# InternetMaximalism/plonky2_bn254

Hardware: AMD Instinct MI355X
Metric: G1 scalar-mul STARK proofs/sec (256-bit scalars) (higher is better)
Workload: dtype u64 (Goldilocks p = 2^64-2^32+1; BN254 Fq as 10x26-bit Montgomery limbs); 1 GPU; configs[1]: batch of 1024 G1 scalar-muls on 1 GPU per step = 8 proofs x 128 instances, 2^16 rows, W=781, standard_fast_config; instances_per_proof=128, steps_in_flight=4, parallelism=1 GPU, no collective

## Files before the change

include/bn254_stark.h:

```cpp
#ifndef BN254_STARK_H
#define BN254_STARK_H

#include <stddef.h>
#include <stdint.h>

#ifdef __cplusplus
extern "C" {
#endif

#define BN254S_ABI_VERSION 1

enum {
  BN254S_OK = 0,
  BN254S_E_INVALID_ARG = -1,
  BN254S_E_HIP = -2,
  BN254S_E_OOM = -3,
  BN254S_E_INVALID_POINT = -4,
  BN254S_E_UNSUPPORTED = -5,
  BN254S_E_TRANSCRIPT = -6,
  BN254S_E_INTERNAL = -7,
  BN254S_E_VERIFY = -8
};

typedef struct bn254s_ctx bn254s_ctx;
// ... 30 lines not shown
                       const uint64_t* offset, size_t n_total, size_t per_proof, bn254s_proof** proofs_out);

typedef struct bn254s_batch bn254s_batch;
int bn254s_prove_batch_begin(bn254s_ctx* ctx, int kind, const bn254s_params* params, const uint64_t* scalars, const uint64_t* x,
                             const uint64_t* offset, size_t n_total, size_t per_proof, bn254s_proof** proofs_out,
                             bn254s_batch** handle);
int bn254s_prove_batch_end(bn254s_batch* handle);

int bn254s_prove_batch_multi(bn254s_ctx** ctxs, size_t n_ctx, int kind, const bn254s_params* params, const uint64_t* scalars,
                             const uint64_t* x, const uint64_t* offset, size_t n_total, size_t per_proof, bn254s_proof** proofs);

int bn254s_prove_g2(bn254s_ctx* ctx, const bn254s_params* params, const uint64_t* scalars, const uint64_t* x,
                    const uint64_t* offset, size_t n, bn254s_proof** out);
int bn254s_prove_fq_exp(bn254s_ctx* ctx, const bn254s_params* params, const uint64_t* scalars ,
                        const uint64_t* x , size_t n, bn254s_proof** out);

int bn254s_proof_words(const bn254s_proof* p, const uint64_t** data, size_t* len);
enum {
  BN254S_SEC_TRACE_CAP = 0,
  BN254S_SEC_AUX_CAP = 1,
  BN254S_SEC_QUOTIENT_CAP = 2,
  BN254S_SEC_LOCAL_VALUES = 3,
  BN254S_SEC_NEXT_VALUES = 4,
  BN254S_SEC_AUX_POLYS = 5,
  BN254S_SEC_AUX_POLYS_NEXT = 6,
  BN254S_SEC_CTL_ZS_FIRST = 7,
  BN254S_SEC_QUOTIENT_POLYS = 8,
  BN254S_SEC_FRI_CAPS = 9,
  BN254S_SEC_QUERY_ROUNDS = 10,
  BN254S_SEC_FINAL_POLY = 11,
  BN254S_SEC_POW_WITNESS = 12,
  BN254S_SEC_INIT_CHALLENGER_STATE = 13,
  BN254S_SEC_COUNT = 14
};
int bn254s_proof_section(const bn254s_proof* p, int id, const uint64_t** data, size_t* len);
int bn254s_proof_degree_bits(const bn254s_proof* p);
int bn254s_proof_outputs(const bn254s_proof* p, const uint64_t** data, size_t* len);
int bn254s_proof_stage_ms(const bn254s_proof* p, const float** ms, size_t* n_stages);
const char* bn254s_stage_name(size_t stage);
size_t bn254s_proof_serialize(const bn254s_proof* p, uint8_t* buf, size_t cap);
void bn254s_proof_free(bn254s_proof* p);

int bn254s_verify(bn254s_ctx* ctx, int kind, const bn254s_params* params, uint32_t degree_bits, const uint64_t* words,
                  size_t n_words, const uint64_t* scalars, const uint64_t* x, const uint64_t* offset, const uint64_t* outputs,
                  size_t n);
int bn254s_verify_host(int kind, const bn254s_params* params, uint32_t degree_bits, const uint64_t* words, size_t n_words,
                       const uint64_t* scalars, const uint64_t* x, const uint64_t* offset, const uint64_t* outputs, size_t n,
                       char* err_buf, size_t err_cap);

int bn254s_verify_batch(bn254s_ctx* ctx, int kind, const bn254s_params* params, uint32_t degree_bits, const uint64_t* const* words,
                        size_t n_words, const uint64_t* scalars, const uint64_t* x, const uint64_t* offset, const uint64_t* outputs,
                        const size_t* n_jobs, size_t n_proofs, int32_t* status, char* err, size_t err_stride);

int bn254s_ctl_values(int kind, const uint64_t* scalars, const uint64_t* x, const uint64_t* offset, const uint64_t* outputs,
                      size_t n, uint64_t* in_rows, uint64_t* out_rows);

int bn254s_map_to_g2(bn254s_ctx* ctx, const bn254s_params* params, const uint64_t* u, const uint64_t* offsets, size_t n,
                     uint64_t* out_points, uint64_t* fq_jobs, uint64_t* g2_jobs, bn254s_proof** fq_proofs,
                     bn254s_proof** g2_proofs);

int bn254s_hash_to_fq2(const uint64_t* input, size_t len, uint64_t* out );
int bn254s_hash_to_fq2_batch(bn254s_ctx* ctx, const uint64_t* inputs, size_t n, size_t len, uint64_t* out);

int bn254s_g1_msm_chain(bn254s_ctx* ctx, const uint64_t* scalars , const uint64_t* x ,
                        const uint64_t* offset , size_t n, uint64_t* offsets_out, uint64_t* result );
int bn254s_g1_msm(bn254s_ctx* ctx, const bn254s_params* params, const uint64_t* scalars, const uint64_t* x,
                  const uint64_t* offset, size_t n, size_t per_proof, uint64_t* result, uint64_t* offsets_out,
                  bn254s_proof** proofs);
int bn254s_g2_msm_chain(bn254s_ctx* ctx, const uint64_t* scalars , const uint64_t* x ,
                        const uint64_t* offset , size_t n, uint64_t* offsets_out ,
                        uint64_t* result );
int bn254s_g2_msm(bn254s_ctx* ctx, const bn254s_params* params, const uint64_t* scalars, const uint64_t* x,
                  const uint64_t* offset, size_t n, size_t per_proof, uint64_t* result, uint64_t* offsets_out,
                  bn254s_proof** proofs);

int bn254s_g1_recover_from_x_batch(bn254s_ctx* ctx, const uint64_t* xs , size_t n,
                                   uint64_t* points_out , uint8_t* flags_out ,
                                   uint64_t* fq_jobs );
int bn254s_g1_recover_from_x(bn254s_ctx* ctx, const bn254s_params* params, const uint64_t* xs, size_t n, size_t per_proof,
                             uint64_t* points_out, uint8_t* flags_out, uint64_t* fq_jobs ,
                             bn254s_proof** fq_proofs);
int bn254s_g2_recover_from_x_batch(bn254s_ctx* ctx, const uint64_t* xs ,
                                   const uint8_t* sgns , size_t n,
                                   uint64_t* points_out , uint8_t* flags_out ,
                                   uint64_t* fq_jobs );
int bn254s_g2_recover_from_x(bn254s_ctx* ctx, const bn254s_params* params, const uint64_t* xs, const uint8_t* sgns, size_t n,
                             size_t per_proof, uint64_t* points_out, uint8_t* flags_out, uint64_t* fq_jobs ,
                             bn254s_proof** fq_proofs);
int bn254s_g2_subgroup_check_batch(bn254s_ctx* ctx, const uint64_t* points , size_t n,
                                   uint8_t* flags_out );
int bn254s_g2_subgroup_check(bn254s_ctx* ctx, const bn254s_params* params, const uint64_t* points ,
                             const uint64_t* offsets , size_t n, size_t per_proof, uint8_t* flags_out ,
                             uint64_t* g2_jobs , bn254s_proof** g2_proofs);
int bn254s_g2_clear_cofactor_batch(bn254s_ctx* ctx, const uint64_t* points , size_t n,
                                   uint64_t* images_out , uint8_t* finite_out );
int bn254s_g2_clear_cofactor(bn254s_ctx* ctx, const bn254s_params* params, const uint64_t* points ,
                             const uint64_t* offsets , size_t n, size_t per_proof, uint64_t* images_out ,
                             uint8_t* finite_out , uint64_t* g2_jobs ,
                             bn254s_proof** g2_proofs);
int bn254s_map_to_g2_batch(bn254s_ctx* ctx, const uint64_t* u , size_t n,
                           uint64_t* out_points );
int bn254s_hash_to_g2_batch(bn254s_ctx* ctx, const uint64_t* inputs , size_t n, size_t len,
                            uint64_t* out_points );
int bn254s_hash_to_fq(const uint64_t* input, size_t len, uint64_t* out );
int bn254s_hash_to_fq_batch(bn254s_ctx* ctx, const uint64_t* inputs, size_t n, size_t len, uint64_t* out );
int bn254s_map_to_g1_batch(bn254s_ctx* ctx, const uint64_t* u , size_t n,
                           uint64_t* out_points , uint8_t* sq_flags ,
                           uint64_t* fq_jobs );
int bn254s_hash_to_g1_batch(bn254s_ctx* ctx, const uint64_t* inputs , size_t n, size_t len,
                            uint64_t* out_points );
int bn254s_map_to_g1(bn254s_ctx* ctx, const bn254s_params* params, const uint64_t* u , size_t n, size_t per_proof,
                     uint64_t* out_points , uint8_t* sq_flags ,
                     uint64_t* fq_jobs , bn254s_proof** fq_proofs );
int bn254s_job_outputs_batch(bn254s_ctx* ctx, int kind, const uint64_t* scalars , const uint64_t* x,
                             const uint64_t* offset, size_t n, uint64_t* outputs_out ,
                             uint8_t* finite_out );
int bn254s_job_outputs(bn254s_ctx* ctx, int kind, const bn254s_params* params, const uint64_t* scalars, const uint64_t* x,
                       const uint64_t* offset, size_t n, size_t per_proof, uint64_t* outputs_out, bn254s_proof** proofs_out);
int bn254s_commit_values(bn254s_ctx* ctx, const uint64_t* values, size_t ncols, uint64_t* coeffs, uint64_t* lde,
                         uint64_t* cap);
int bn254s_bench_ntt(bn254s_ctx* ctx, size_t ncols, int iters, float* ms);
int bn254s_bench_ntt_clock(bn254s_ctx* ctx, size_t ncols, int iters, float* ms, float* mhz, float* mhz_min);
int bn254s_bench_issue(bn254s_ctx* ctx, float* ns_per_issue, float* mhz);
int bn254s_bench_copy(bn254s_ctx* ctx, size_t words, int iters);
int bn254s_bench_leafhash(bn254s_ctx* ctx, size_t ncols, int log_leaves, int iters, float* ms);
int bn254s_poseidon_permute(bn254s_ctx* ctx, uint64_t* states, size_t n);
int bn254s_selftest_field(bn254s_ctx* ctx, const uint64_t* a, const uint64_t* b, size_t n, uint64_t* out);
int bn254s_selftest_poseidon(bn254s_ctx* ctx, int variant, uint64_t* states, size_t n);
int bn254s_selftest_leaf_hash(bn254s_ctx* ctx, const uint64_t* data, size_t ncols, int log_leaves, int kernel, int chunk_cols,
                              uint64_t* digests);
int bn254s_selftest_fq_inv(bn254s_ctx* ctx, const uint64_t* x, size_t n, uint64_t* out);
int bn254s_selftest_fq(bn254s_ctx* ctx, int group, const uint64_t* in, size_t n, uint64_t* out);
int bn254s_selftest_logup(bn254s_ctx* ctx, const uint64_t* trace, size_t rows, int ncols, int rc_begin, int n_rc, int table_col,
                          int freq_col, const uint64_t betas[2], uint64_t* out);
int bn254s_selftest_acc(bn254s_ctx* ctx, const uint64_t* values, const uint64_t* weights, size_t T, size_t rows, uint64_t* out);
int bn254s_selftest_openings(bn254s_ctx* ctx, const uint64_t* coeffs, int npolys, int log_r, const uint64_t zeta[2],
                             const uint64_t zeta_next[2], uint64_t* out);
int bn254s_selftest_fri_combine(bn254s_ctx* ctx, int mode, int W, int n_rc, int n_ctl, size_t n, const uint64_t* cols,
                                const uint64_t* aux_in, const uint64_t* points, uint64_t* out);
int bn254s_selftest_fri_fold(bn254s_ctx* ctx, const uint64_t* in, int log_m, uint64_t shift, const uint64_t beta[2], uint64_t* out);
int bn254s_selftest_fri_rows(bn254s_ctx* ctx, const uint64_t* lde, int ncols, int log_n, int h, size_t k0, size_t rows,
                             const uint32_t* indices, int nq, uint64_t* window, uint64_t* gathered);
#define BN254S_VERIFY_RECORD_HEAD 34
int bn254s_selftest_verify_front(int kind, const bn254s_params* params, uint32_t degree_bits, const uint64_t* words, size_t n_words,
                                 uint64_t* record_out, size_t record_cap);
int bn254s_selftest_query_round(bn254s_ctx* ctx, int kind, const bn254s_params* params, uint32_t degree_bits,
                                const uint64_t* const* words, size_t n_words, const uint64_t* records, size_t n_proofs,
                                size_t chunk_proofs, int32_t* codes_out);
const char* bn254s_selftest_query_text(int n_layers, int code);
int bn254s_selftest_verify_batch_ms(bn254s_ctx* ctx, float ms_out[5]);
#define BN254S_PLAN_WORDS 54
int bn254s_selftest_proof_plan(int kind, size_t n, const bn254s_params* params, uint64_t dev_total_bytes, int force_split,
                               int force_lowmem, int force_stream, int stream_win_log, uint64_t* out, char* err, size_t err_len);
int bn254s_generate_trace(bn254s_ctx* ctx, int kind, const uint64_t* scalars, const uint64_t* x, const uint64_t* offset,
                          size_t n, uint32_t min_rows_log2, uint64_t* trace_out, uint64_t* outputs);
int bn254s_g1_generate_trace(bn254s_ctx* ctx, const uint64_t* scalars, const uint64_t* x, const uint64_t* offset,
                             size_t n, uint32_t min_rows_log2, uint64_t* trace_out, uint64_t* outputs);

#ifdef __cplusplus
}
#endif
#endif
```

plonky2_bn254_amd/__init__.py:

```python
import os as _os

_os.environ.setdefault("GPU_MAX_HW_QUEUES", "16")

from .lib import Context, Proof, load_library, LibraryMissing, VerifyError, default_params, proof_plan, proof_words, prove_batch_multi, query_round, query_text, verify_g1_msm, verify_g1_recover, verify_g2_clear_cofactor, verify_g2_msm, verify_g2_recover, verify_batch_host, verify_front, verify_g2_subgroup, verify_host, verify_job_outputs, verify_map_to_g1
```

plonky2_bn254_amd/csrc/capi.hip:

```cpp
#include <algorithm>
#include <cstring>
#include "proven_jobs.h"
#include "merkle.h"
#include "trace_g1.h"
#include "fq_selftest.h"
#include "aux.h"
#include "poseidon_dev.h"

void ntt_module_warm();
void merkle_module_warm();
void aux_module_warm();
void fri_module_warm();
void quotient_g1_module_warm();
void quotient_g2fq_module_warm();
void trace_g1_module_warm();
void trace_g2fq_module_warm();
void prover_module_warm();

extern "C" {

int bn254s_abi_version(void) { return BN254S_ABI_VERSION; }

void bn254s_params_default(bn254s_params* p) {
  p->struct_size = sizeof(bn254s_params);
  p->security_bits = 100;
  p->num_challenges = 2;
  p->rate_bits = 1;
  p->cap_height = 4;
  p->pow_bits = 16;
  p->arity_bits = 4;
  p->final_poly_bits = 5;
  p->num_queries = 84;
  p->min_rows_log2 = 16;
}

__attribute__((constructor)) static void bn254s_runtime_defaults() { setenv("GPU_MAX_HW_QUEUES", "16", 0); }


int bn254s_ctx_create(int device_id, bn254s_ctx** out) {
  if (!out) return BN254S_E_INVALID_ARG;
  *out = nullptr;
  int ndev = 0;
  if (hipGetDeviceCount(&ndev) != hipSuccess || device_id < 0 || device_id >= ndev) return BN254S_E_HIP;
  if (const char* e = getenv("BN254S_SYNC"))
    if (!strcmp(e, "blocking")) (void)hipSetDeviceFlags(hipDeviceScheduleBlockingSync);
  (void)hipGetLastError();
  if (hipSetDevice(device_id) != hipSuccess) return BN254S_E_HIP;
  bn254s_ctx* c = new bn254s_ctx();
  c->device = device_id;
  merkle_set_throughput_mode(getenv("BN254S_COOP_MAX_NODES") ? atol(getenv("BN254S_COOP_MAX_NODES")) : -1,
                             getenv("BN254S_MERKLE_LEVEL_ASM") ? atoi(getenv("BN254S_MERKLE_LEVEL_ASM")) : -1);
  if (const char* e = getenv("BN254S_BIG_CAP")) c->big_cap = std::max(1, atoi(e));
  if (const char* e = getenv("BN254S_SCHED_FIFO")) c->big_fifo = atoi(e) != 0;
  if (const char* e = getenv("BN254S_NTT_CONVOY")) c->big_convoy = std::max(0, atoi(e));
  if (const char* e = getenv("BN254S_HASH_SPLIT")) c->hash_split = std::min(8, std::max(1, atoi(e)));
  c->big_cost[BIG_NTT] = c->big_cap;
  const char* cost_env[3] = {"BN254S_BIG_COST_NTT", "BN254S_BIG_COST_EXCL", "BN254S_BIG_COST_HASH"};
  for (int k = 0; k < 3; k++) {
    if (const char* e = getenv(cost_env[k])) c->big_cost[k] = atoi(e);
    c->big_cost[k] = std::min(c->big_cap, std::max(0, c->big_cost[k]));
  }
  c->big_cost[BIG_HASH_PART] = std::max(1, c->big_cost[BIG_HASH] / c->hash_split);
  if (hipStreamCreateWithFlags(&c->stream, hipStreamNonBlocking) != hipSuccess) {
    delete c;
    return BN254S_E_HIP;
  }
  if (ntt_tables_init(&c->ntt) != 0) {
    delete c;
    return BN254S_E_OOM;
  }
  {
    void* h = nullptr;
    if (hipHostMalloc(&h, 256 << 10) == hipSuccess) {
      (void)hipMemcpyAsync(h, c->ntt.twmat_fwd, 256 << 10, hipMemcpyDeviceToHost, c->stream);
      (void)hipStreamSynchronize(c->stream);
      hipHostFree(h);
    }
  }
  ntt_module_warm();
  merkle_module_warm();
  aux_module_warm();
  fri_module_warm();
  quotient_g1_module_warm();
  quotient_g2fq_module_warm();
  trace_g1_module_warm();
  trace_g2fq_module_warm();
  prover_module_warm();
  *out = c;
  return BN254S_OK;
}

void bn254s_ctx_destroy(bn254s_ctx* c) {
  if (!c) return;
  hipSetDevice(c->device);
  c->workers.shutdown();
  hipStreamSynchronize(c->stream);
  for (Slot* s : c->slots) {
    hipStreamSynchronize(s->st);
    s->mem.release();
    if (s->pinned) hipHostFree(s->pinned);
    for (auto& e : s->events) hipEventDestroy(e);
    hipStreamDestroy(s->st);
    delete s;
  }
  for (auto& kv : c->tall) {
    ntt_tall_tables_free(kv.second);
    delete kv.second;
  }
  for (auto& kv : c->split) {
    ntt_split_tables_free(kv.second);
    delete kv.second;
  }
  c->release();
  ntt_tables_free(&c->ntt);
  hipStreamDestroy(c->stream);
  delete c;
}

int bn254s_ctx_trim(bn254s_ctx* c) {
  if (!c) return BN254S_E_INVALID_ARG;
  HIP_TRY(c, hipSetDevice(c->device));
  auto give_back = [&](size_t i) {
    if (i < c->n_slots_now()) c->slot(i)->mem.release();
  };
  if (c->workers.busy.empty()) {
    for (size_t i = 0; i < c->n_slots_now(); i++) give_back(i);
  } else {
    c->workers.for_idle_slots(give_back);
  }
  bool idle;
  {
    std::lock_guard<std::mutex> lk(c->workers.mu);
    idle = c->workers.n_busy == 0 && c->workers.q.empty();
  }
  if (idle) {
    HIP_TRY(c, hipStreamSynchronize(c->stream));
    c->release();
  }
  return BN254S_OK;
}

const char* bn254s_last_error(const bn254s_ctx* c) { return c ? c->err.c_str() : "null context"; }

int bn254s_commit_values(bn254s_ctx* c, const uint64_t* values, size_t ncols, uint64_t* coeffs, uint64_t* lde,
                         uint64_t* cap) {
  if (!c || !values || ncols == 0) return BN254S_E_INVALID_ARG;
  HIP_TRY(c, hipSetDevice(c->device));
  const size_t N = NTT_N;
  u64* d_vals = c->words("cv.vals", ncols * N);
  u64* d_tmp = c->words("cv.tmp", 3 * ncols * N);
  u64* d_lde = c->words("cv.lde", ncols * 2 * N);
  u64* d_tree = c->words("cv.tree", merkle_tree_digests(17, 4) * 4);
  if (!d_vals || !d_tmp || !d_lde || !d_tree) return BN254S_E_OOM;
  HIP_TRY(c, hipMemcpyAsync(d_vals, values, ncols * N * 8, hipMemcpyHostToDevice, c->stream));
  ntt_inverse_lde(&c->ntt, d_vals, d_vals, d_lde, d_tmp, d_tmp + ncols * N, (int)ncols, c->stream);
  merkle_build(d_lde, 1, 2 * N, (int)ncols, 17, 4, d_tree, c->stream);
  HIP_TRY(c, hipGetLastError());
  if (coeffs) HIP_TRY(c, hipMemcpyAsync(coeffs, d_vals, ncols * N * 8, hipMemcpyDeviceToHost, c->stream));
  if (lde) HIP_TRY(c, hipMemcpyAsync(lde, d_lde, ncols * 2 * N * 8, hipMemcpyDeviceToHost, c->stream));
  if (cap)
    HIP_TRY(c, hipMemcpyAsync(cap, d_tree + 4 * merkle_level_offset(17, 13), 16 * 32, hipMemcpyDeviceToHost, c->stream));
  HIP_TRY(c, hipStreamSynchronize(c->stream));
  return BN254S_OK;
}

__global__ void k_fill_pseudo(u64* p, size_t n, u64 seed) {
  size_t i = (size_t)blockIdx.x * blockDim.x + threadIdx.x;
  if (i >= n) return;
  u64 z = seed + i * 0x9E3779B97F4A7C15ULL;
  z = (z ^ (z >> 30)) * 0xBF58476D1CE4E5B9ULL;
  z = (z ^ (z >> 27)) * 0x94D049BB133111EBULL;
  z ^= z >> 31;
  p[i] = z >= GL_P ? z - GL_P : z;
}

int bn254s_bench_ntt(bn254s_ctx* c, size_t ncols, int iters, float* ms) {
  if (!c || !ms || ncols == 0 || iters <= 0) return BN254S_E_INVALID_ARG;
  HIP_TRY(c, hipSetDevice(c->device));
  const size_t N = NTT_N;
  u64* d_vals = c->words("cv.vals", ncols * N);
  u64* d_tmp = c->words("cv.tmp", 3 * ncols * N);
  u64* d_lde = c->words("cv.lde", ncols * 2 * N);
  if (!d_vals || !d_tmp || !d_lde) return BN254S_E_OOM;
  size_t n = ncols * N;
  k_fill_pseudo<<<(unsigned)((n + 255) / 256), 256, 0, c->stream>>>(d_vals, n, 0x1234);
  hipEvent_t e0, e1;
  HIP_TRY(c, hipEventCreate(&e0));
  HIP_TRY(c, hipEventCreate(&e1));
  ntt_inverse_lde(&c->ntt, d_vals, d_vals, d_lde, d_tmp, d_tmp + n, (int)ncols, c->stream);
  HIP_TRY(c, hipEventRecord(e0, c->stream));
  for (int it = 0; it < iters; it++) ntt_inverse_lde(&c->ntt, d_vals, d_vals, d_lde, d_tmp, d_tmp + n, (int)ncols, c->stream);
  HIP_TRY(c, hipEventRecord(e1, c->stream));
  HIP_TRY(c, hipEventSynchronize(e1));
  float t = 0;
  HIP_TRY(c, hipEventElapsedTime(&t, e0, e1));
  *ms = t / iters;
  hipEventDestroy(e0);
  hipEventDestroy(e1);
  HIP_TRY(c, hipGetLastError());
  return BN254S_OK;
}

__global__ __launch_bounds__(64) void k_clock_probe(unsigned long long* __restrict__ samples, const int* __restrict__ stop, int max_samples,
                                                    int* __restrict__ n_taken) {
  if (threadIdx.x != 0) return;
  int i = 0;
  for (; i < max_samples; i++) {
    samples[2 * i] = __builtin_readcyclecounter();
    samples[2 * i + 1] = __builtin_amdgcn_s_memrealtime();
    if (__hip_atomic_load(stop, __ATOMIC_RELAXED, __HIP_MEMORY_SCOPE_AGENT)) {
      i++;
      break;
    }
    __builtin_amdgcn_s_sleep(127);
    __builtin_amdgcn_s_sleep(127);
    __builtin_amdgcn_s_sleep(127);
  }
  *n_taken = i;
}
__global__ __launch_bounds__(256) void k_issue_probe(u64* out) {
  for (int i = 0; i < 2048; i++) {
    asm volatile(
        "v_lshl_add_u64 v[40:41], v[40:41], 0, v[48:49]\n v_lshl_add_u64 v[42:43], v[42:43], 0, v[48:49]\n"
        "v_lshl_add_u64 v[44:45], v[44:45], 0, v[48:49]\n v_lshl_add_u64 v[46:47], v[46:47], 0, v[48:49]\n"
        "v_lshl_add_u64 v[40:41], v[40:41], 0, v[48:49]\n v_lshl_add_u64 v[42:43], v[42:43], 0, v[48:49]\n"
        "v_lshl_add_u64 v[44:45], v[44:45], 0, v[48:49]\n v_lshl_add_u64 v[46:47], v[46:47], 0, v[48:49]\n"
        "v_lshl_add_u64 v[40:41], v[40:41], 0, v[48:49]\n v_lshl_add_u64 v[42:43], v[42:43], 0, v[48:49]\n"
        "v_lshl_add_u64 v[44:45], v[44:45], 0, v[48:49]\n v_lshl_add_u64 v[46:47], v[46:47], 0, v[48:49]\n"
        "v_lshl_add_u64 v[40:41], v[40:41], 0, v[48:49]\n v_lshl_add_u64 v[42:43], v[42:43], 0, v[48:49]\n"
        "v_lshl_add_u64 v[44:45], v[44:45], 0, v[48:49]\n v_lshl_add_u64 v[46:47], v[46:47], 0, v[48:49]\n"
        "v_lshl_add_u64 v[40:41], v[40:41], 0, v[48:49]\n v_lshl_add_u64 v[42:43], v[42:43], 0, v[48:49]\n"
        "v_lshl_add_u64 v[44:45], v[44:45], 0, v[48:49]\n v_lshl_add_u64 v[46:47], v[46:47], 0, v[48:49]\n"
        "v_lshl_add_u64 v[40:41], v[40:41], 0, v[48:49]\n v_lshl_add_u64 v[42:43], v[42:43], 0, v[48:49]\n"
        "v_lshl_add_u64 v[44:45], v[44:45], 0, v[48:49]\n v_lshl_add_u64 v[46:47], v[46:47], 0, v[48:49]\n"
        "v_lshl_add_u64 v[40:41], v[40:41], 0, v[48:49]\n v_lshl_add_u64 v[42:43], v[42:43], 0, v[48:49]\n"
        "v_lshl_add_u64 v[44:45], v[44:45], 0, v[48:49]\n v_lshl_add_u64 v[46:47], v[46:47], 0, v[48:49]\n"
        "v_lshl_add_u64 v[40:41], v[40:41], 0, v[48:49]\n v_lshl_add_u64 v[42:43], v[42:43], 0, v[48:49]\n"
        "v_lshl_add_u64 v[44:45], v[44:45], 0, v[48:49]\n v_lshl_add_u64 v[46:47], v[46:47], 0, v[48:49]\n" ::
            : "v40", "v41", "v42", "v43", "v44", "v45", "v46", "v47");
  }
  u32 a;
  asm volatile("v_mov_b32 %0, v40" : "=v"(a));
  out[(size_t)blockIdx.x * blockDim.x + threadIdx.x] = a;
}
int bn254s_bench_issue(bn254s_ctx* c, float* ns_per_issue, float* mhz) {
  if (!c || !ns_per_issue || !mhz) return BN254S_E_INVALID_ARG;
  HIP_TRY(c, hipSetDevice(c->device));
  hipDeviceProp_t prop;
  HIP_TRY(c, hipGetDeviceProperties(&prop, c->device));
  const int simds = prop.multiProcessorCount * 4, blocks = simds * 8 / 4;
  const int MAXS = 20000;
  u64* d_out = c->words("iss.out", (size_t)blocks * 256);
  unsigned long long* d_s = (unsigned long long*)c->words("clk.samples", 2 * (size_t)MAXS + 2);
  if (!d_out || !d_s) return BN254S_E_OOM;
  int* d_flags = (int*)(d_s + 2 * (size_t)MAXS);
  hipStream_t ps = nullptr;
  HIP_TRY(c, hipStreamCreateWithFlags(&ps, hipStreamNonBlocking));
  HIP_TRY(c, hipMemsetAsync(d_flags, 0, 8, c->stream));
  HIP_TRY(c, hipStreamSynchronize(c->stream));
  hipEvent_t e0, e1;
  HIP_TRY(c, hipEventCreate(&e0));
  HIP_TRY(c, hipEventCreate(&e1));
  k_clock_probe<<<1, 64, 0, ps>>>(d_s, d_flags, MAXS, d_flags + 1);
  const int reps = 12;
  for (int i = 0; i < 4; i++) k_issue_probe<<<blocks, 256, 0, c->stream>>>(d_out);
  HIP_TRY(c, hipEventRecord(e0, c->stream));
  for (int i = 0; i < reps; i++) k_issue_probe<<<blocks, 256, 0, c->stream>>>(d_out);
  HIP_TRY(c, hipEventRecord(e1, c->stream));
  (void)hipMemsetAsync(d_flags, 1, 1, c->stream);
  HIP_TRY(c, hipStreamSynchronize(c->stream));
  (void)hipStreamSynchronize(ps);
  hipStreamDestroy(ps);
  float t = 0;
  HIP_TRY(c, hipEventElapsedTime(&t, e0, e1));
  hipEventDestroy(e0);
  hipEventDestroy(e1);
  *ns_per_issue = (float)((double)t * 1e6 / reps / (2048.0 * 32 * 8));
  std::vector<unsigned long long> h(2 * (size_t)MAXS + 2);
  HIP_TRY(c, hipMemcpy(h.data(), d_s, h.size() * 8, hipMemcpyDeviceToHost));
  const int n = ((const int*)&h[2 * (size_t)MAXS])[1];
  *mhz = 0;
  if (n >= 8) {
    const int lo = n / 4;
    const double dt = (double)(h[2 * (size_t)(n - 1) + 1] - h[2 * (size_t)lo + 1]), dc = (double)(h[2 * (size_t)(n - 1)] - h[2 * (size_t)lo]);
    if (dt > 0) *mhz = (float)(dc / dt * 100.0);
  }
  return BN254S_OK;
}

int bn254s_bench_ntt_clock(bn254s_ctx* c, size_t ncols, int iters, float* ms, float* mhz, float* mhz_min) {
  if (!c || !ms || !mhz || ncols == 0 || iters <= 0) return BN254S_E_INVALID_ARG;
  HIP_TRY(c, hipSetDevice(c->device));
  const int MAXS = 20000;
  unsigned long long* d_s = (unsigned long long*)c->words("clk.samples", 2 * (size_t)MAXS + 2);
  if (!d_s) return BN254S_E_OOM;
// ... 263 lines not shown
```

plonky2_bn254_amd/csrc/ctx.h:

```cpp
#pragma once
#include <string>
#include <vector>
#include <map>
#include <cstdio>
#include <mutex>
#include <condition_variable>
#include <chrono>
#include <deque>
#include <functional>
#include <thread>
#include <atomic>
#include <hip/hip_runtime.h>
#include "../../include/bn254_stark.h"
#include "gl_dev.h"
#include "ntt.h"

struct BufPool {
  std::map<std::string, std::pair<void*, size_t>> pool;
  std::string err;
  void* buf(const std::string& name, size_t bytes) {
    auto it = pool.find(name);
    if (it != pool.end() && it->second.second >= bytes) return it->second.first;
    if (it != pool.end()) {
      hipFree(it->second.first);
      pool.erase(it);
    }
    void* p = nullptr;
    if (hipMalloc(&p, bytes) != hipSuccess) {
      (void)hipGetLastError();
      err = "hipMalloc failed for " + name + " (" + std::to_string(bytes) + " bytes)";
      return nullptr;
    }
    pool[name] = {p, bytes};
    return p;
  }
  u64* words(const std::string& name, size_t n) { return (u64*)buf(name, n * 8); }
  bool has(const std::string& name) const { return pool.find(name) != pool.end(); }
  void drop(const std::string& name) {
    auto it = pool.find(name);
    if (it == pool.end()) return;
    hipFree(it->second.first);
    pool.erase(it);
  }
  void release() {
    for (auto& kv : pool) hipFree(kv.second.first);
    pool.clear();
  }
};

struct Slot {
  hipStream_t st = nullptr;
  BufPool mem;
  void* pinned = nullptr;
  size_t pinned_bytes = 0;
  std::vector<hipEvent_t> events;
};

enum { BIG_NTT = 0, BIG_EXCL = 1, BIG_HASH = 2, BIG_HASH_PART = 3 };

struct WorkPool {
  std::mutex mu;
  std::condition_variable cv, done_cv;
  std::deque<std::function<void(size_t)>> q;
  std::vector<std::thread> th;
  std::vector<char> busy;
  bool stop = false;
  size_t limit = 0, n_busy = 0;
  size_t n_waiting = 0, completions = 0;
  std::mutex retry_mu;
  std::atomic<int> in_flight{0};
  void start(size_t n, int device) {
    std::lock_guard<std::mutex> lk(mu);
    limit = n;
    if (busy.size() < n) busy.resize(n, 0);
    while (th.size() < n) {
      th.emplace_back([this, device]() {
        (void)hipSetDevice(device);
        for (;;) {
          std::function<void(size_t)> f;
          size_t s = 0;
          {
            std::unique_lock<std::mutex> lk2(mu);
            auto free_slot = [&]() -> size_t {
              for (size_t i = 0; i < limit && i < busy.size(); i++)
                if (!busy[i]) return i;
              return (size_t)-1;
            };
            cv.wait(lk2, [&] { return (stop && q.empty()) || (!q.empty() && n_busy < limit && free_slot() != (size_t)-1); });
            if (q.empty()) return;
            f = std::move(q.front());
            q.pop_front();
            s = free_slot();
            busy[s] = 1;
            n_busy++;
            in_flight.store((int)n_busy, std::memory_order_relaxed);
          }
          f(s);
          {
            std::lock_guard<std::mutex> lk3(mu);
            busy[s] = 0;
            n_busy--;
            in_flight.store((int)n_busy, std::memory_order_relaxed);
            completions++;
          }
          cv.notify_one();
          done_cv.notify_all();
        }
      });
    }
  }
  void push(std::function<void(size_t)> f) {
    {
      std::lock_guard<std::mutex> lk(mu);
      q.push_back(std::move(f));
    }
    cv.notify_one();
  }
  template <class G>
  void for_idle_slots(G g) {
    std::vector<size_t> idle;
    {
      std::lock_guard<std::mutex> lk(mu);
      for (size_t i = 0; i < busy.size(); i++)
        if (!busy[i]) {
          busy[i] = 2;
          idle.push_back(i);
        }
    }
    for (size_t i : idle) g(i);
    {
      std::lock_guard<std::mutex> lk(mu);
      for (size_t i : idle) busy[i] = 0;
    }
    cv.notify_all();
  }
  size_t active() {
    std::lock_guard<std::mutex> lk(mu);
    return n_busy - n_waiting;
  }
  size_t completions_now() {
    std::lock_guard<std::mutex> lk(mu);
    return completions;
  }
  void wait_for_a_completion(size_t c0) {
    std::unique_lock<std::mutex> lk(mu);
    n_waiting++;
    done_cv.wait_for(lk, std::chrono::seconds(60), [&] { return completions != c0; });
    n_waiting--;
  }
  void shutdown() {
    {
      std::lock_guard<std::mutex> lk(mu);
      stop = true;
    }
    cv.notify_all();
    for (auto& t : th) t.join();
    th.clear();
  }
};

struct bn254s_ctx : BufPool {
  int device = 0;
  hipStream_t stream = nullptr;
  NttTables ntt;
  std::vector<Slot*> slots;
  WorkPool workers;
  std::map<unsigned, NttTallTables*> tall;
  std::map<unsigned, NttSplitTables*> split;
  std::mutex big_mu;
  std::condition_variable big_cv;
  int big_cap = 12, big_cost[4] = {12, 2, 4, 2}, big_used = 0;
  int hash_split = 1;
  bool big_fifo = true;
  struct BigWaiter {
    unsigned long id;
    int cls;
  };
  std::deque<BigWaiter> big_q;
  unsigned long big_next_id = 0;
  int big_convoy = 4, big_convoy_run = 0;
  bool big_last_was_ntt = false;
  void big_lock(int cls) {
    std::unique_lock<std::mutex> lk(big_mu);
    if (big_fifo) {
      const unsigned long my = big_next_id++;
      big_q.push_back({my, cls});
      big_cv.wait(lk, [&] {
        if (big_q.front().id == my) {
          if (big_used + big_cost[cls] > big_cap) return false;
          if (big_last_was_ntt && cls != BIG_NTT && big_convoy_run < big_convoy)
            for (const BigWaiter& w : big_q)
              if (w.cls == BIG_NTT) return false;
          return true;
        }
        if (cls != BIG_NTT || !big_last_was_ntt || big_used != 0 || big_convoy_run >= big_convoy) return false;
        if (big_q.front().cls == BIG_NTT) return false;
        for (const BigWaiter& w : big_q) {
          if (w.cls == BIG_NTT) return w.id == my;
        }
        return false;
      });
      const bool in_order = big_q.front().id == my;
      for (auto it = big_q.begin(); it != big_q.end(); ++it)
        if (it->id == my) {
          big_q.erase(it);
          break;
        }
      if (in_order) big_convoy_run = 0;
      else big_convoy_run++;
      big_last_was_ntt = false;
      big_used += big_cost[cls];
      lk.unlock();
      big_cv.notify_all();
      return;
    }
    big_cv.wait(lk, [&] { return big_used + big_cost[cls] <= big_cap; });
    big_used += big_cost[cls];
  }
  void big_unlock(int cls) {
    {
      std::lock_guard<std::mutex> lk(big_mu);
      big_used -= big_cost[cls];
      big_last_was_ntt = cls == BIG_NTT && big_used == 0;
    }
    big_cv.notify_all();
  }
  static constexpr size_t MAX_SLOTS = 64;
  std::mutex slots_mu, err_mu;
  float vb_ms[5] = {0, 0, 0, 0, 0};
  bn254s_ctx() { slots.reserve(MAX_SLOTS); }
  void set_err(const std::string& e) {
    std::lock_guard<std::mutex> lk(err_mu);
    err = e;
  }
  size_t n_slots_now() {
    std::lock_guard<std::mutex> lk(slots_mu);
    return slots.size();
  }
  Slot* slot(size_t i) {
    if (i >= MAX_SLOTS) return nullptr;
    std::lock_guard<std::mutex> lk(slots_mu);
    while (slots.size() <= i) {
      Slot* s = new Slot();
      if (hipStreamCreateWithFlags(&s->st, hipStreamNonBlocking) != hipSuccess) {
        delete s;
        return nullptr;
      }
      slots.push_back(s);
    }
    return slots[i];
  }
};

#define HIP_TRY(ctx, call)                                                                  \
  do {                                                                                      \
    hipError_t e_ = (call);                                                                 \
    if (e_ != hipSuccess) {                                                                 \
      (ctx)->set_err(std::string(#call) + ": " + hipGetErrorString(e_));                    \
      return BN254S_E_HIP;                                                                  \
    }                                                                                       \
  } while (0)
```

plonky2_bn254_amd/csrc/ntt.h:

```cpp
#pragma once
#include <vector>
#include "gl_dev.h"

static constexpr size_t NTT_N = 65536;

struct NttTables {
  u64 *tw256_fwd = nullptr, *tw256_inv = nullptr;
  u64 *twmat_fwd = nullptr, *twmat_inv = nullptr;
  u64* twmat_inv_ninv = nullptr;
  u64* coset_pow[2] = {nullptr, nullptr};
  u64* coset_inv_pow[2] = {nullptr, nullptr};
  u64 n_inv = 0;
};

int ntt_tables_init(NttTables* T);
void ntt_tables_free(NttTables* T);
void ntt_inverse(const NttTables* T, const u64* values, u64* coeffs, u64* tmp, int ncols, hipStream_t s);
void ntt_coset_inverse(const NttTables* T, int h, const u64* values, u64* coeffs, u64* tmp, int ncols, hipStream_t s);
void ntt_lde(const NttTables* T, const u64* coeffs, u64* lde, u64* tmp, int ncols, hipStream_t s);
void ntt_inverse_lde(const NttTables* T, const u64* values, u64* coeffs, u64* lde, u64* tmp, u64* tmp2, int ncols, hipStream_t s);
void ntt_coset_forward_natural(const NttTables* T, int h, const u64* coeffs, u64* values, u64* tmp, int ncols, hipStream_t s);

struct NttTallTables {
  unsigned log_n = 0;
  u64* wn_inv_pow = nullptr;
  u64* wn_pow_br = nullptr;
  u64* block_coset_pow[2] = {nullptr, nullptr};
  u64 shift[2] = {0, 0};
  u64 r_inv = 0;
};
int ntt_tall_tables_init(NttTallTables* T, unsigned log_n, u64 base_shift = GL_GEN);
void ntt_tall_tables_free(NttTallTables* T);
void ntt_inverse_tall(const NttTables* T, const NttTallTables* TT, const u64* values, u64* coeffs, u64* tmp, int ncols,
                      hipStream_t s);
void ntt_coset_inverse_tall(const NttTables* T, const NttTallTables* TT, int h, const u64* values, u64* coeffs, u64* tmp, int ncols,
                            hipStream_t s);
void ntt_inverse_lde_tall(const NttTables* T, const NttTallTables* TT, const u64* values, u64* coeffs, u64* lde, u64* tmp, int ncols,
                          hipStream_t s);
void ntt_lde_tall(const NttTables* T, const NttTallTables* TT, const u64* coeffs, u64* lde, u64* tmp, int ncols, hipStream_t s,
                  int coset_mask = 3);

struct NttSplitTables {
  unsigned log_n = 0;
  u64 *fwd_lo = nullptr, *fwd_hi = nullptr, *inv_lo = nullptr, *inv_hi = nullptr;
  u64 shift[2] = {0, 0};
  u64 half = 0;
};
int ntt_split_tables_init(NttSplitTables* S, unsigned log_n);
void ntt_split_tables_free(NttSplitTables* S);
void ntt_split_inverse(const NttSplitTables* S, const u64* values, u64* halves, int ncols, hipStream_t s);
void ntt_split_forward(const NttSplitTables* S, const u64* eo, u64* lde, size_t lde_stride, int ncols, hipStream_t s, int coset_mask = 3);
void ntt_coset_inverse_split(const NttTables* T, const NttTallTables* TT, const NttSplitTables* S, int h, const u64* values, u64* coeffs,
                             u64* tmp, int ncols, hipStream_t s);

static constexpr int FIELD_SELFTEST_OUTS = 17;
void field_selftest(const u64* a, const u64* b, u64* out, size_t n, hipStream_t s);
```

plonky2_bn254_amd/csrc/ntt.hip:

```cpp
#include "gl_dev.h"
#include "gl_asm.h"
#include "ntt.h"

#if defined(__HIP_DEVICE_COMPILE__) && defined(BN254S_NTT_PRIO) && BN254S_NTT_PRIO > 0
#define NTT_KERNEL_PRIO() __builtin_amdgcn_s_setprio(BN254S_NTT_PRIO)
#else
#define NTT_KERNEL_PRIO() ((void)0)
#endif

template <bool INV, int SPAN, int G, int J>
__device__ __forceinline__ void bfly16(u64* x) {
  constexpr int E = J * (8 / SPAN);
  constexpr int S0 = E == 0 ? 0 : (!INV ? 12 * E : 192 - 12 * E);
  constexpr bool NEG0 = S0 >= 96;
  constexpr int S1 = NEG0 ? S0 - 96 : S0;
  constexpr bool RIGHT = S1 > 64;
  constexpr bool NEG = NEG0 != RIGHT;
  u64 s, d;
  gl_bfly_asm<NEG>(x[G + J], x[G + J + SPAN], s, d);
  x[G + J] = s;
  if constexpr (S1 == 0) x[G + J + SPAN] = d;
  else if constexpr (RIGHT) x[G + J + SPAN] = gl_shr_small_asm<96 - S1>(d);
  else x[G + J + SPAN] = gl_shl_asm<S1>(d);
}
// ... 122 lines not shown
    __syncthreads();
    ulonglong2* o16 = reinterpret_cast<ulonglong2*>(ocol + (size_t)br4(blockIdx.x) * 16 * 256);
#pragma unroll
    for (int i = 0; i < 8; i++) {
      const int piece = i * 256 + t;
      o16[piece] = stage[(piece >> 7) * STAGE_ROW + ((piece >> 3) & 15) * 9 + (piece & 7)];
    }
  } else {
#pragma unroll
    for (int kb = 0; kb < 16; kb++) {
      int k = k1 + 256 * (ka + 16 * kb);
      u64 v = x[br4(kb)];
      if (post) v = gl_mul_asm(v, post[k]);
      else if (post_scalar != 1) v = gl_mul_asm(v, post_scalar);
      ocol[k] = v;
    }
  }
}

template <int NPARK>
__global__ __launch_bounds__(256, NPARK ? 4 : 3) void k_ntt_intt2_lde1(const u64* __restrict__ in, size_t in_stride, u64* __restrict__ coef,
                                                        size_t coef_stride, u64* __restrict__ y0, u64* __restrict__ y1,
                                                        size_t y_stride, const u64* __restrict__ tw256_inv,
                                                        const u64* __restrict__ pre0, const u64* __restrict__ pre1,
                                                        const u64* __restrict__ twmat, const u64* __restrict__ tw256_fwd,
                                                        unsigned log_r) {
  NTT_KERNEL_PRIO();
  __shared__ u32 lds[LDS_TILE_WORDS];
  __shared__ u64 park[NPARK ? NPARK * 256 : 1];
  u64 c[16];
  const int t = threadIdx.x;
  int g = t & 15, d = t >> 4;
  const u64* col = in + col_offset(blockIdx.y, log_r, in_stride);
  u64 x[16];
  {
    const int k1_load = blockIdx.x * 16 + d;
#pragma unroll
    for (int m = 0; m < 16; m++) x[m] = col[k1_load * 256 + g + 16 * m];
  }
  dft256_tile<true, 2>(x, lds, tw256_inv, d, g);
  const int i2 = blockIdx.x * 16 + d;
  u64* ocol = coef + col_offset(blockIdx.y, log_r, coef_stride);
#pragma unroll
  for (int kb = 0; kb < 16; kb++) {
    c[kb] = x[br4(kb)];
    ocol[i2 + 256 * (g + 16 * kb)] = c[kb];
    if (kb >= 16 - NPARK) park[(kb - (16 - NPARK)) * 256 + t] = c[kb];
  }
#pragma unroll 1
  for (int h = 0; h < 2; h++) {
    const u64* __restrict__ pre = h ? pre1 : pre0;
    u64* ycol = (h ? y1 : y0) + col_offset(blockIdx.y, log_r, y_stride);
    asm volatile("" : "+v"(g), "+v"(d));
#pragma unroll
    for (int m = 0; m < 16; m++) {
      x[m] = gl_mul_asm(m >= 16 - NPARK ? park[(m - (16 - NPARK)) * 256 + t] : c[m], pre[(g + 16 * m) * 256 + i2]);
      if ((m & 3) == 3) __builtin_amdgcn_sched_barrier(0);
    }
    __syncthreads();
    dft256_tile<false, 0>(x, lds, tw256_fwd, d, g);
#pragma unroll
    for (int kb = 0; kb < 16; kb++) {
      int k1 = g + 16 * kb;
      ycol[k1 * 256 + i2] = gl_mul_asm(x[br4(kb)], twmat[k1 * 256 + i2]);
      if ((kb & 3) == 3) __builtin_amdgcn_sched_barrier(0);
    }
  }
}

static void fill_pow_table(std::vector<u64>& t, u64 base, size_t n, u64 first = 1) {
  t.resize(n);
  u64 v = first;
  for (size_t i = 0; i < n; i++) {
    t[i] = v;
    v = gl_mul(v, base);
  }
}

int ntt_tables_init(NttTables* T) {
  const size_t N = NTT_N;
  std::vector<u64> h;
  auto upload = [&](u64** dst, const std::vector<u64>& src) -> int {
    if (hipMalloc((void**)dst, src.size() * 8) != hipSuccess) return -1;
    if (hipMemcpy(*dst, src.data(), src.size() * 8, hipMemcpyHostToDevice) != hipSuccess) return -1;
    return 0;
  };
  u64 wN = gl_root_of_unity(16), wNi = gl_inv(wN);
  u64 w256 = gl_root_of_unity(8), w256i = gl_inv(w256);
  fill_pow_table(h, w256, 256);
  if (upload(&T->tw256_fwd, h)) return -1;
  fill_pow_table(h, w256i, 256);
  if (upload(&T->tw256_inv, h)) return -1;
  for (int inv = 0; inv < 2; inv++) {
    u64 w = inv ? wNi : wN;
    h.resize(N);
    u64 wk = 1;
    for (int k1 = 0; k1 < 256; k1++) {
      u64 v = 1;
      for (int i2 = 0; i2 < 256; i2++) {
        h[k1 * 256 + i2] = v;
        v = gl_mul(v, wk);
      }
      wk = gl_mul(wk, w);
    }
    if (upload(inv ? &T->twmat_inv : &T->twmat_fwd, h)) return -1;
    if (inv) {
      const u64 ninv0 = gl_inv((u64)N);
      for (auto& v : h) v = gl_mul(v, ninv0);
      if (upload(&T->twmat_inv_ninv, h)) return -1;
    }
  }
  u64 w2N = gl_root_of_unity(17);
  u64 shifts[2] = {GL_GEN, gl_mul(GL_GEN, w2N)};
  u64 ninv = gl_inv((u64)N);
  for (int hh = 0; hh < 2; hh++) {
    fill_pow_table(h, shifts[hh], N);
    if (upload(&T->coset_pow[hh], h)) return -1;
    fill_pow_table(h, gl_inv(shifts[hh]), N, ninv);
    if (upload(&T->coset_inv_pow[hh], h)) return -1;
  }
  T->n_inv = ninv;
  return 0;
}

void ntt_tables_free(NttTables* T) {
  hipFree(T->tw256_fwd);
  hipFree(T->tw256_inv);
  hipFree(T->twmat_fwd);
  hipFree(T->twmat_inv);
  hipFree(T->twmat_inv_ninv);
  for (int h = 0; h < 2; h++) {
    hipFree(T->coset_pow[h]);
    hipFree(T->coset_inv_pow[h]);
  }
}

void ntt_inverse(const NttTables* T, const u64* values, u64* coeffs, u64* tmp, int ncols, hipStream_t s) {
  dim3 grid(16, ncols), block(256);
  k_ntt_pass1<true><<<grid, block, 0, s>>>(values, NTT_N, tmp, NTT_N, nullptr, T->twmat_inv, T->tw256_inv, 0);
  k_ntt_pass2<true, false><<<grid, block, 0, s>>>(tmp, NTT_N, coeffs, NTT_N, nullptr, T->n_inv, T->tw256_inv, 0);
}
void ntt_coset_inverse(const NttTables* T, int h, const u64* values, u64* coeffs, u64* tmp, int ncols, hipStream_t s) {
  dim3 grid(16, ncols), block(256);
  k_ntt_pass1<true><<<grid, block, 0, s>>>(values, NTT_N, tmp, NTT_N, nullptr, T->twmat_inv, T->tw256_inv, 0);
  k_ntt_pass2<true, false><<<grid, block, 0, s>>>(tmp, NTT_N, coeffs, NTT_N, T->coset_inv_pow[h], 1, T->tw256_inv, 0);
}
void ntt_lde(const NttTables* T, const u64* coeffs, u64* lde, u64* tmp, int ncols, hipStream_t s) {
  dim3 grid(16, ncols), block(256);
  for (int h = 0; h < 2; h++) {
    k_ntt_pass1<false><<<grid, block, 0, s>>>(coeffs, NTT_N, tmp, NTT_N, T->coset_pow[h], T->twmat_fwd, T->tw256_fwd, 0);
    k_ntt_pass2<false, true><<<grid, block, 0, s>>>(tmp, NTT_N, lde + (size_t)h * NTT_N, 2 * NTT_N, nullptr, 1, T->tw256_fwd, 0);
  }
}
void ntt_inverse_lde(const NttTables* T, const u64* values, u64* coeffs, u64* lde, u64* tmp, u64* tmp2, int ncols, hipStream_t s) {
  dim3 grid(16, ncols), block(256);
  u64* y0 = tmp2;
  u64* y1 = tmp2 + (size_t)ncols * NTT_N;
  k_ntt_pass1<true><<<grid, block, 0, s>>>(values, NTT_N, tmp, NTT_N, nullptr, T->twmat_inv_ninv, T->tw256_inv, 0);
  k_ntt_intt2_lde1<8><<<grid, block, 0, s>>>(tmp, NTT_N, coeffs, NTT_N, y0, y1, NTT_N, T->tw256_inv, T->coset_pow[0],
                                          T->coset_pow[1], T->twmat_fwd, T->tw256_fwd, 0);
  k_ntt_pass2<false, true><<<grid, block, 0, s>>>(y0, NTT_N, lde, 2 * NTT_N, nullptr, 1, T->tw256_fwd, 0);
  k_ntt_pass2<false, true><<<grid, block, 0, s>>>(y1, NTT_N, lde + NTT_N, 2 * NTT_N, nullptr, 1, T->tw256_fwd, 0);
}
void ntt_coset_forward_natural(const NttTables* T, int h, const u64* coeffs, u64* values, u64* tmp, int ncols, hipStream_t s) {
  dim3 grid(16, ncols), block(256);
  k_ntt_pass1<false><<<grid, block, 0, s>>>(coeffs, NTT_N, tmp, NTT_N, T->coset_pow[h], T->twmat_fwd, T->tw256_fwd, 0);
  k_ntt_pass2<false, false><<<grid, block, 0, s>>>(tmp, NTT_N, values, NTT_N, nullptr, 1, T->tw256_fwd, 0);
}


__device__ __forceinline__ u64 mul_2exp3(u64 x, int e) {
  switch (e) {
    case 0: return x;
    case 1: return gl_mul_2exp<3>(x);
    case 2: return gl_mul_2exp<6>(x);
    case 3: return gl_mul_2exp<9>(x);
    case 4: return gl_mul_2exp<12>(x);
    case 5: return gl_mul_2exp<15>(x);
    case 6: return gl_mul_2exp<18>(x);
    case 7: return gl_mul_2exp<21>(x);
    case 8: return gl_mul_2exp<24>(x);
    case 9: return gl_mul_2exp<27>(x);
    case 10: return gl_mul_2exp<30>(x);
    case 11: return gl_mul_2exp<33>(x);
    case 12: return gl_mul_2exp<36>(x);
    case 13: return gl_mul_2exp<39>(x);
    case 14: return gl_mul_2exp<42>(x);
    case 15: return gl_mul_2exp<45>(x);
    case 16: return gl_mul_2exp<48>(x);
    case 17: return gl_mul_2exp<51>(x);
    case 18: return gl_mul_2exp<54>(x);
    case 19: return gl_mul_2exp<57>(x);
    case 20: return gl_mul_2exp<60>(x);
    case 21: return gl_mul_2exp<63>(x);
    case 22: return gl_mul_2exp<66>(x);
    case 23: return gl_mul_2exp<69>(x);
    case 24: return gl_mul_2exp<72>(x);
    case 25: return gl_mul_2exp<75>(x);
    case 26: return gl_mul_2exp<78>(x);
    case 27: return gl_mul_2exp<81>(x);
    case 28: return gl_mul_2exp<84>(x);
    case 29: return gl_mul_2exp<87>(x);
    case 30: return gl_mul_2exp<90>(x);
    case 31: return gl_mul_2exp<93>(x);
    case 32: return gl_mul_2exp<96>(x);
    case 33: return gl_mul_2exp<99>(x);
    case 34: return gl_mul_2exp<102>(x);
    case 35: return gl_mul_2exp<105>(x);
    case 36: return gl_mul_2exp<108>(x);
    case 37: return gl_mul_2exp<111>(x);
    case 38: return gl_mul_2exp<114>(x);
    case 39: return gl_mul_2exp<117>(x);
    case 40: return gl_mul_2exp<120>(x);
    case 41: return gl_mul_2exp<123>(x);
    case 42: return gl_mul_2exp<126>(x);
    case 43: return gl_mul_2exp<129>(x);
    case 44: return gl_mul_2exp<132>(x);
    case 45: return gl_mul_2exp<135>(x);
    case 46: return gl_mul_2exp<138>(x);
    case 47: return gl_mul_2exp<141>(x);
    case 48: return gl_mul_2exp<144>(x);
    case 49: return gl_mul_2exp<147>(x);
    case 50: return gl_mul_2exp<150>(x);
    case 51: return gl_mul_2exp<153>(x);
    case 52: return gl_mul_2exp<156>(x);
    case 53: return gl_mul_2exp<159>(x);
    case 54: return gl_mul_2exp<162>(x);
    case 55: return gl_mul_2exp<165>(x);
    case 56: return gl_mul_2exp<168>(x);
    case 57: return gl_mul_2exp<171>(x);
    case 58: return gl_mul_2exp<174>(x);
    case 59: return gl_mul_2exp<177>(x);
    case 60: return gl_mul_2exp<180>(x);
    case 61: return gl_mul_2exp<183>(x);
    case 62: return gl_mul_2exp<186>(x);
    default: return gl_mul_2exp<189>(x);
  }
}
template <int LOGR, bool INV>
__device__ __forceinline__ void dft_small(u64* x) {
  constexpr int R = 1 << LOGR;
#pragma unroll
  for (int s = 0; s < LOGR; s++) {
    const int span = R >> (s + 1);
#pragma unroll
    for (int g0 = 0; g0 < R; g0 += 2 * span) {
#pragma unroll
      for (int jj = 0; jj < span; jj++) {
        u64 a = x[g0 + jj], b = x[g0 + jj + span];
        x[g0 + jj] = gl_add(a, b);
        int e = (jj << s) * (64 >> LOGR);
        if (INV) e = (64 - e) & 63;
        x[g0 + jj + span] = mul_2exp3(gl_sub(a, b), e);
      }
    }
  }
}
__device__ __forceinline__ constexpr int brn(int v, int bits) {
  int r = 0;
  for (int i = 0; i < bits; i++) r |= ((v >> i) & 1) << (bits - 1 - i);
  return r;
}

template <int LOGR>
__global__ __launch_bounds__(256) void k_ntt_outer_inv(const u64* __restrict__ in, u64* __restrict__ out, size_t N,
                                                       const u64* __restrict__ wn_inv_pow , u64 r_inv) {
  constexpr int R = 1 << LOGR;
  const size_t i2 = (size_t)blockIdx.x * blockDim.x + threadIdx.x;
  const u64* c = in + (size_t)blockIdx.y * N;
  u64* o = out + (size_t)blockIdx.y * N;
  u64 x[R];
#pragma unroll
  for (int i1 = 0; i1 < R; i1++) x[i1] = c[(size_t)i1 * NTT_N + i2];
  dft_small<LOGR, true>(x);
  const u64 w = wn_inv_pow[i2];
  u64 f = r_inv;
#pragma unroll
  for (int k1 = 0; k1 < R; k1++) {
    o[(size_t)k1 * NTT_N + i2] = gl_mul(x[brn(k1, LOGR)], f);
    f = gl_mul(f, w);
  }
}

template <int LOGR>
__global__ __launch_bounds__(256) void k_ntt_outer_fwd(const u64* __restrict__ z, size_t N, u64* __restrict__ out,
                                                       size_t out_stride, const u64* __restrict__ wn_pow_br ,
                                                       u64 shift) {
  constexpr int R = 1 << LOGR;
  const size_t p = (size_t)blockIdx.x * blockDim.x + threadIdx.x;
  const u64* c = z + (size_t)blockIdx.y * N;
  u64 x[R];
  const u64 b = gl_mul(shift, wn_pow_br[p]);
  u64 f = 1;
#pragma unroll
  for (int i1 = 0; i1 < R; i1++) {
    u64 v = c[(size_t)i1 * NTT_N + p];
    x[i1] = i1 ? gl_mul(v, f) : v;
    f = gl_mul(f, b);
  }
  dft_small<LOGR, false>(x);
  constexpr int CH = R < 16 ? R : 16;
  constexpr int U = CH / 2;
  constexpr int PITCH = U + 1;
  __shared__ ulonglong2 stage[256 * PITCH];
  const int t = threadIdx.x;
  ulonglong2* o16 = reinterpret_cast<ulonglong2*>(out + (size_t)blockIdx.y * out_stride + (size_t)blockIdx.x * 256 * R);
#pragma unroll
  for (int c0 = 0; c0 < R; c0 += CH) {
    if (c0) __syncthreads();
#pragma unroll
    for (int u = 0; u < U; u++) {
      ulonglong2 w2;
      w2.x = x[c0 + 2 * u];
      w2.y = x[c0 + 2 * u + 1];
// ... 264 lines not shown
```

plonky2_bn254_amd/csrc/prover.hip:

```cpp
#include <algorithm>
#include <atomic>
#include <cstring>
#include <thread>
#include "ctx.h"
#include "trace_g1.h"
#include "trace_g2fq.h"
#include "aux.h"
#include "merkle.h"
#include "quotient.h"
#include "fri.h"
#include "transcript.h"
#include "prover.h"
#include "proof_plan.h"

template <class L>
static StarkShape make_shape(bool input_has_a, int n_constraints) {
  StarkShape s;
  s.W = L::W;
  s.rc_begin = L::RC_BEGIN;
  s.rc_end = L::RC_END;
  s.table_col = L::RANGE;
  s.freq_col = L::FREQ;
  s.n_ctl = 2;
  s.n_constraints = n_constraints;
  memset(&s.ctl, 0, sizeof(s.ctl));
  int m = 0;
  for (int i = 0; i < L::PL; i++, m++) { s.ctl.col_start[0][m] = L::B + i; s.ctl.col_bits[0][m] = 1; }
  if (input_has_a)
    for (int i = 0; i < L::PL; i++, m++) { s.ctl.col_start[0][m] = L::A + i; s.ctl.col_bits[0][m] = 1; }
  for (int k = 0; k < 16; k++, m++) { s.ctl.col_start[0][m] = L::BITS + 16 * k; s.ctl.col_bits[0][m] = 16; }
  s.ctl.col_start[0][m] = L::TIMESTAMP; s.ctl.col_bits[0][m] = 1; m++;
  s.ctl.ncols[0] = m;
  s.ctl.filter_col[0] = L::FLAGS + 0;
  m = 0;
  for (int i = 0; i < L::PL; i++, m++) { s.ctl.col_start[1][m] = L::SUM + i; s.ctl.col_bits[1][m] = 1; }
  s.ctl.col_start[1][m] = L::TIMESTAMP; s.ctl.col_bits[1][m] = 1; m++;
  s.ctl.ncols[1] = m;
  s.ctl.filter_col[1] = L::FLAGS + 1;
  return s;
}
static int fq_generate_trace_no_offset(const u64* d_scalars, const u64* d_x, const u64*, size_t n, u64* d_trace, size_t N,
                                       u64* d_scratch, u64* d_outputs, int* d_err, hipStream_t st, bool with_range) {
  return fq_generate_trace_device(d_scalars, d_x, n, d_trace, N, d_scratch, d_outputs, d_err, st, with_range);
}
const StarkKind& stark_kind(int kind) {
  static const StarkKind kinds[3] = {
      {make_shape<G1L>(true, 1111), 8, true, g1_trace_scratch_words, g1_generate_trace_device, g1_quotient_mz_blocks, g1_quotient_launch},
      {make_shape<G2L>(true, 1693), 16, true, g2_trace_scratch_words, g2_generate_trace_device, g2_quotient_mz_blocks, g2_quotient_launch},
      {make_shape<FQL>(false, 770), 4, false, fq_trace_scratch_words, fq_generate_trace_no_offset, fq_quotient_mz_blocks, fq_quotient_launch}};
  return kinds[kind];
}

enum { ST_TRACE = 0, ST_TRACE_NTT, ST_TRACE_MERKLE, ST_AUX, ST_AUX_NTT, ST_AUX_MERKLE, ST_QUOTIENT, ST_QUOTIENT_COMMIT,
       ST_OPENINGS, ST_FRI, ST_TOTAL, ST_COUNT };
static const char* STAGE_NAMES[ST_COUNT] = {"trace_gen", "trace_ntt", "trace_merkle", "aux_columns", "aux_ntt", "aux_merkle",
                                            "quotient", "quotient_commit", "openings", "fri", "total"};

struct bn254s_proof {
  std::vector<u64> words, outputs;
  size_t sec_off[BN254S_SEC_COUNT + 1] = {0};
  int degree_bits = 0;
  float stage_ms[ST_COUNT] = {0};
};

std::vector<int> fri_arities(const bn254s_params& P, int degree_bits) {
  std::vector<int> a;
  int d = degree_bits;
  while (d > (int)P.final_poly_bits && d + (int)P.rate_bits - (int)P.arity_bits >= (int)P.cap_height) {
    a.push_back(P.arity_bits);
    d -= P.arity_bits;
  }
  return a;
}

__global__ __launch_bounds__(256) void k_quotient_chunks(const u64* __restrict__ ab, u64* __restrict__ out, size_t N, u64 inv2,
                                                         u64 inv2c) {
  size_t i = (size_t)blockIdx.x * blockDim.x + threadIdx.x;
  if (i >= N) return;
  int a = blockIdx.y;
  u64 A = ab[(size_t)(a * 2 + 0) * N + i], B = ab[(size_t)(a * 2 + 1) * N + i];
  out[(size_t)(a * 2 + 0) * N + i] = gl_mul(gl_add(A, B), inv2);
  out[(size_t)(a * 2 + 1) * N + i] = gl_mul(gl_sub(A, B), inv2c);
}

#define CHK(call)                                              \
  do {                                                         \
    hipError_t e_ = (call);                                    \
    if (e_ != hipSuccess) {                                    \
      err = std::string(#call) + ": " + hipGetErrorString(e_); \
      return BN254S_E_HIP;                                     \
    }                                                          \
  } while (0)

static const NttTallTables* get_tall_tables(bn254s_ctx* c, unsigned log_n, bool half_of_split = false) {
  static std::mutex mu;
  std::lock_guard<std::mutex> lk(mu);
  const unsigned key = log_n + (half_of_split ? 100 : 0);
  auto it = c->tall.find(key);
  if (it != c->tall.end()) return it->second;
  NttTallTables* t = new NttTallTables();
  if (ntt_tall_tables_init(t, log_n, half_of_split ? gl_mul(GL_GEN, GL_GEN) : GL_GEN) != 0) {
    delete t;
    return nullptr;
  }
  c->tall[key] = t;
  return t;
}
static const NttSplitTables* get_split_tables(bn254s_ctx* c, unsigned log_n) {
  static std::mutex mu;
  std::lock_guard<std::mutex> lk(mu);
  auto it = c->split.find(log_n);
  if (it != c->split.end()) return it->second;
  NttSplitTables* t = new NttSplitTables();
  if (ntt_split_tables_init(t, log_n) != 0) {
    delete t;
    return nullptr;
  }
  c->split[log_n] = t;
  return t;
}

struct BigSection {
  bn254s_ctx* c;
  hipStream_t st;
  int cls;
  BigSection(bn254s_ctx* c_, hipStream_t st_, int cls_) : c(c_), st(st_), cls(cls_) { c->big_lock(cls); }
  ~BigSection() {
    hipStreamSynchronize(st);
    c->big_unlock(cls);
  }
};

static int get_point_tables(bn254s_ctx* c, unsigned log_n, QPointTables& pt) {
  static std::mutex mu;
  std::lock_guard<std::mutex> lk(mu);
  std::string key = "pt." + std::to_string(log_n);
  bool fresh = !c->has(key);
  size_t M2 = (size_t)2 << log_n;
  u64* p = c->words(key, 3 * M2);
  if (!p) return BN254S_E_OOM;
  if (fresh) {
    quotient_point_tables(p, p + M2, p + 2 * M2, log_n, c->stream);
    if (hipStreamSynchronize(c->stream) != hipSuccess) return BN254S_E_HIP;
  }
  pt.x = p;
  pt.lfirst = p + M2;
  pt.llast = p + 2 * M2;
  return 0;
}

struct Workspace {
  Slot* sl = nullptr;
  const ProofPlan* pl = nullptr;
  u64 *in, *tvals, *tcoef, *hist, *tmp, *ldechunk, *sponge, *comb, *tlde, *trees, *avals, *acoef, *alde, *scr, *quot, *tabs, *open,
      *fri, *fritrees, *qout;
  int* err;
  unsigned long long* pow;
  u32* qidx;
  u64 *ttree, *atree, *qtree;
  u64 *qv, *ab, *qcoef, *qlde, *qpart;
  u64 *W, *mzt, *apow;
  size_t cap_off;
  u64 *tw = nullptr, *aw = nullptr, *wpt = nullptr, *qrows = nullptr;
  int begin_windows(std::string& err);
};

static int workspace_acquire(Slot& sl, const ProofPlan& pl, Workspace& ws, std::string& err) {
  BufPool& mem = sl.mem;
  const PlanBuffers& b = pl.words;
  const bool stream = pl.stream, lowmem = pl.lowmem;
  ws.sl = &sl;
  ws.pl = &pl;
  if (lowmem) {
    mem.drop("acoef");
    mem.drop("alde");
  }
  ws.in = mem.words("in", b.in);
  ws.tvals = mem.words("tvals", b.tvals);
  ws.tcoef = mem.words("tcoef", b.tcoef);
  ws.hist = mem.words("hist", b.hist);
  ws.tmp = mem.words("tmp", b.tmp);
  mem.drop("win");
  if (stream) {
    mem.drop("tlde");
    mem.drop("alde");
    mem.drop("acoef");
  } else {
    mem.drop("ldechunk");
    mem.drop("sponge");
  }
  ws.ldechunk = stream ? mem.words("ldechunk", b.ldechunk) : nullptr;
  ws.sponge = stream ? mem.words("sponge", b.sponge) : nullptr;
  ws.comb = mem.words("comb", b.comb);
  ws.tlde = stream ? ws.ldechunk : mem.words("tlde", b.tlde);
  ws.trees = mem.words("trees", b.trees);
  ws.avals = mem.words("avals", b.avals);
  ws.acoef = lowmem ? ws.avals : mem.words("acoef", b.acoef);
  ws.alde = stream ? ws.ldechunk : lowmem ? ws.tvals : mem.words("alde", b.alde);
  ws.scr = mem.words("scratch", b.scratch);
  ws.quot = mem.words("quot", b.quot);
  ws.tabs = mem.words("tabs", b.tabs);
  ws.open = mem.words("open", b.open);
  ws.fri = mem.words("fri", b.fri);
  ws.fritrees = mem.words("fritrees", b.fritrees);
  ws.qout = mem.words("qout", b.qout);
  if (sl.pinned_bytes < pl.pinned_bytes) {
    if (sl.pinned) hipHostFree(sl.pinned);
    sl.pinned = nullptr;
    sl.pinned_bytes = 0;
    CHK(hipHostMalloc(&sl.pinned, pl.pinned_bytes));
    sl.pinned_bytes = pl.pinned_bytes;
  }
  if (!ws.hist || !ws.in || !ws.tvals || !ws.tcoef || !ws.tmp || !ws.tlde || !ws.trees || !ws.avals || !ws.acoef || !ws.alde ||
      !ws.scr || !ws.quot || !ws.tabs || !ws.open || !ws.fri || !ws.fritrees || !ws.qout || !ws.comb ||
      (stream && (!ws.ldechunk || !ws.sponge))) {
    err = mem.err;
    mem.release();
    return BN254S_E_OOM;
  }
  {
    static const size_t reserve = (size_t)(getenv("BN254S_MEM_RESERVE_MB") ? atol(getenv("BN254S_MEM_RESERVE_MB")) : 6144) << 20;
    size_t free_b = 0, total_b = 0;
    if (hipMemGetInfo(&free_b, &total_b) == hipSuccess && free_b < reserve) {
      err = "device memory: " + std::to_string(free_b >> 20) + " MB would be left free, below the reserve of " +
            std::to_string(reserve >> 20) + " MB kept for the runtime's own allocations";
      mem.release();
      return BN254S_E_OOM;
    }
  }
  const size_t N = pl.N, M2 = pl.M2;
  const int NQ = ProofPlan::NQ;
  ws.err = (int*)(ws.in + pl.in_words);
  ws.pow = (unsigned long long*)(ws.in + pl.in_words + 2);
  ws.qidx = (u32*)(ws.qout + pl.n_q());
  ws.ttree = ws.trees;
  ws.atree = ws.trees + pl.tree_words;
  ws.qtree = ws.trees + 2 * pl.tree_words;
  ws.qv = ws.quot;
  ws.ab = ws.quot + (size_t)NQ * N;
  ws.qcoef = ws.quot + (size_t)2 * NQ * N;
  ws.qlde = ws.quot + (size_t)3 * NQ * N;
  ws.qpart = ws.qlde + (size_t)NQ * M2;
  ws.W = ws.tabs;
  ws.mzt = ws.tabs + QUOTIENT_W_WORDS(pl.K);
  ws.apow = ws.mzt + QUOTIENT_MZT_WORDS;
  ws.cap_off = 4 * merkle_level_offset(pl.log_m2, pl.log_m2 - pl.P.cap_height);
  return BN254S_OK;
}

int Workspace::begin_windows(std::string& err) {
  BufPool& mem = sl->mem;
  const size_t WROWS = pl->WROWS;
  CHK(hipStreamSynchronize(sl->st));
  mem.drop("tvals");
  tvals = nullptr;
  u64* win = mem.words("win", pl->words.win);
  if (!win) {
    err = mem.err;
    mem.release();
    return BN254S_E_OOM;
  }
  tw = win;
  aw = win + (size_t)pl->W * WROWS;
  wpt = aw + (size_t)pl->A * WROWS;
  qrows = wpt + 3 * WROWS;
  return BN254S_OK;
}

struct Transforms {
  static constexpr int CH = ProofPlan::CH;
  bn254s_ctx* c;
  hipStream_t st;
  const NttTallTables* TT;
  const NttSplitTables* SP;
  const ProofPlan& pl;
  u64 *tmp, *ldechunk, *sponge;
  u64* eo() const { return tmp; }
  u64* ntmp() const { return tmp + (size_t)CH * 2 * pl.N; }

  void commit_ntt(const u64* vals, u64* coef, u64* lde, int nc) const {
    const size_t N = pl.N, M2 = pl.M2;
    if (pl.log_s) {
      for (int c0 = 0; c0 < nc; c0 += CH) {
        const int cn = std::min(CH, nc - c0);
        ntt_split_inverse(SP, vals + (size_t)c0 * N, coef + (size_t)c0 * N, cn, st);
        ntt_inverse_lde_tall(&c->ntt, TT, coef + (size_t)c0 * N, coef + (size_t)c0 * N, eo(), ntmp(), 2 * cn, st);
        ntt_split_forward(SP, eo(), lde + (size_t)c0 * M2, M2, cn, st);
      }
    } else if (pl.log_r && pl.lowmem) {
      for (int c0 = 0; c0 < nc; c0 += CH) {
        const int cn = std::min(CH, nc - c0);
        ntt_inverse_lde_tall(&c->ntt, TT, vals + (size_t)c0 * N, coef + (size_t)c0 * N, lde + (size_t)c0 * M2, tmp, cn, st);
      }
    } else if (pl.log_r) {
      ntt_inverse_lde_tall(&c->ntt, TT, vals, coef, lde, tmp, nc, st);
    } else {
      ntt_inverse_lde(&c->ntt, vals, coef, lde, tmp, tmp + (size_t)nc * N, nc, st);
    }
  }
  void lde(const u64* coef, u64* out, int nc) const {
    const size_t N = pl.N, M2 = pl.M2;
    if (pl.log_s) {
      for (int c0 = 0; c0 < nc; c0 += CH) {
        const int cn = std::min(CH, nc - c0);
        ntt_lde_tall(&c->ntt, TT, coef + (size_t)c0 * N, eo(), ntmp(), 2 * cn, st);
        ntt_split_forward(SP, eo(), out + (size_t)c0 * M2, M2, cn, st);
      }
    } else if (pl.log_r) ntt_lde_tall(&c->ntt, TT, coef, out, tmp, nc, st);
    else ntt_lde(&c->ntt, coef, out, tmp, nc, st);
  }
  void lde_chunk(const u64* coef, int cn, int coset_mask = 3) const {
    if (pl.log_s) {
      ntt_lde_tall(&c->ntt, TT, coef, eo(), ntmp(), 2 * cn, st, coset_mask);
      ntt_split_forward(SP, eo(), ldechunk, pl.M2, cn, st, coset_mask);
    } else {
      ntt_lde_tall(&c->ntt, TT, coef, ldechunk, tmp, cn, st, coset_mask);
    }
  }
  template <class F>
  void for_lde_chunks(const u64* coef, int nc, int coset_mask, F use) const {
    for (int c0 = 0; c0 < nc; c0 += CH) {
      const int cn = std::min(CH, nc - c0);
      lde_chunk(coef + (size_t)c0 * pl.N, cn, coset_mask);
      use(c0, cn);
    }
  }
  void commit_stream(const u64* vals, u64* coef, int nc, u64* tree) const {
    const size_t N = pl.N, M2 = pl.M2;
    for (int c0 = 0; c0 < nc; c0 += CH) {
      const int cn = std::min(CH, nc - c0);
      if (pl.log_s) {
        ntt_split_inverse(SP, vals + (size_t)c0 * N, coef + (size_t)c0 * N, cn, st);
        ntt_inverse_lde_tall(&c->ntt, TT, coef + (size_t)c0 * N, coef + (size_t)c0 * N, eo(), ntmp(), 2 * cn, st);
        ntt_split_forward(SP, eo(), ldechunk, M2, cn, st);
      } else {
        ntt_inverse_lde_tall(&c->ntt, TT, vals + (size_t)c0 * N, coef + (size_t)c0 * N, ldechunk, tmp, cn, st);
      }
      merkle_absorb(ldechunk, M2, cn, (int)pl.log_m2, sponge, c0 == 0, c0 + cn == nc ? tree : nullptr, st);
    }
  }
  void quotient_coset_inverse(const u64* qv, u64* ab) const {
    const size_t N = pl.N;
    for (int a = 0; a < 2; a++)
      for (int h = 0; h < 2; h++)
        if (pl.log_s) ntt_coset_inverse_split(&c->ntt, TT, SP, h, qv + (size_t)(a * 2 + h) * N, ab + (size_t)(a * 2 + h) * N, tmp, 1, st);
        else if (pl.log_r) ntt_coset_inverse_tall(&c->ntt, TT, h, qv + (size_t)(a * 2 + h) * N, ab + (size_t)(a * 2 + h) * N, tmp, 1, st);
        else ntt_coset_inverse(&c->ntt, h, qv + (size_t)(a * 2 + h) * N, ab + (size_t)(a * 2 + h) * N, tmp, 1, st);
  }
};

struct Run {
  bn254s_ctx* c;
  Slot& sl;
  hipStream_t st;
  const ProofPlan& pl;
  Workspace& ws;
  const Transforms& tf;
  QPointTables pt;
  void sb(int stage) const { hipEventRecord(sl.events[2 * stage], st); }
  void se(int stage) const { hipEventRecord(sl.events[2 * stage + 1], st); }
  int mmode() const { return c->workers.in_flight.load(std::memory_order_relaxed) >= 4 ? MERKLE_THROUGHPUT : MERKLE_LATENCY; }
};

static int upload_and_generate(const StarkKind& sk, const u64* scalars, const u64* x, const u64* off, size_t n, u64* d_in, u64* d_trace,
                               size_t N, u64* d_scr, u64* d_outs, int* d_err, hipStream_t st, bool with_range, std::string& err) {
  const size_t PW = sk.point_words;
  u64* d_sc = d_in;
  u64* d_x = d_in + 4 * n;
  u64* d_off = d_x + PW * n;
  CHK(hipMemcpyAsync(d_sc, scalars, n * 32, hipMemcpyHostToDevice, st));
  CHK(hipMemcpyAsync(d_x, x, n * PW * 8, hipMemcpyHostToDevice, st));
  if (sk.has_offset) CHK(hipMemcpyAsync(d_off, off, n * PW * 8, hipMemcpyHostToDevice, st));
  if (sk.generate_trace(d_sc, d_x, d_off, n, d_trace, N, d_scr, d_outs, d_err, st, with_range)) {
    err = "trace generation launch failed";
    return BN254S_E_HIP;
  }
  return BN254S_OK;
}

static int stage_trace(const Run& r, const u64* scalars, const u64* x, const u64* off, bn254s_proof* pr, int* h_err, std::string& err) {
  const ProofPlan& pl = r.pl;
  const Workspace& ws = r.ws;
  const StarkShape& sh = pl.sh;
  hipStream_t st = r.st;
  r.sb(ST_TRACE);
  CHK(hipMemsetAsync(ws.err, 0, 16, st));
  u64* d_outs = ws.open;
  if (int rc = upload_and_generate(stark_kind(pl.kind), scalars, x, off, pl.n, ws.in, ws.tvals, pl.N, ws.scr, d_outs, ws.err, st, false, err))
    return rc;
  {
    BigSection big(r.c, st, BIG_EXCL);
    launch_range_columns(ws.tvals, pl.N, sh.rc_begin, sh.rc_end, sh.freq_col, sh.table_col, (u32*)ws.hist, ws.err, st);
  }
  pr->outputs.resize(pl.n * (size_t)pl.PW);
  CHK(hipMemcpyAsync(pr->outputs.data(), d_outs, pl.n * (size_t)pl.PW * 8, hipMemcpyDeviceToHost, st));
  CHK(hipMemcpyAsync(h_err, ws.err, 4, hipMemcpyDeviceToHost, st));
  r.se(ST_TRACE);
  return BN254S_OK;
}

static void hash_sections(const Run& r, const u64* lde, int width, u64* tree, int stage) {
  bn254s_ctx* c = r.c;
  const size_t M2 = r.pl.M2;
  const int S = r.pl.log_n == 16 ? c->hash_split : 1;
  if (S <= 1) {
    BigSection big(c, r.st, BIG_HASH);
    r.sb(stage);
    merkle_leaves(lde, 1, M2, width, r.pl.log_m2, tree, r.st);
    return;
  }
  const size_t cnt = M2 / S;
  for (int k = 0; k < S; k++) {
    BigSection big(c, r.st, BIG_HASH_PART);
    if (k == 0) r.sb(stage);
    merkle_leaves_range(lde, 1, M2, width, (size_t)k * cnt, cnt, tree, r.st);
  }
}

static int commit(const Run& r, const u64* vals, u64* coef, u64* lde, int width, u64* tree, int ntt_stage, int merkle_stage,
                  u64* cap_out, std::string& err) {
  const ProofPlan& pl = r.pl;
  hipStream_t st = r.st;
  if (pl.stream) {
    BigSection big(r.c, st, BIG_NTT);
    r.sb(ntt_stage);
    r.tf.commit_stream(vals, coef, width, tree);
    r.se(ntt_stage);
    r.sb(merkle_stage);
  } else {
    {
      BigSection big(r.c, st, BIG_NTT);
      r.sb(ntt_stage);
      r.tf.commit_ntt(vals, coef, lde, width);
      r.se(ntt_stage);
    }
    hash_sections(r, lde, width, tree, merkle_stage);
  }
  merkle_upper(pl.log_m2, pl.P.cap_height, tree, st, r.mmode());
  CHK(hipMemcpyAsync(cap_out, tree + r.ws.cap_off, ProofPlan::CAPW * 8, hipMemcpyDeviceToHost, st));
  r.se(merkle_stage);
  CHK(hipStreamSynchronize(st));
  return BN254S_OK;
}

static void stage_aux(const Run& r, const u64 betas[2], const u64 gammas[2]) {
  BigSection big(r.c, r.st, BIG_EXCL);
  r.sb(ST_AUX);
  aux_build(r.pl.sh, r.ws.tvals, r.pl.N, betas, gammas, r.ws.avals, r.ws.scr, r.ws.err, r.st);
  r.se(ST_AUX);
}

static void quotient_over_windows(const Run& r, const u64 betas[2], const u64 gammas[2]) {
  const ProofPlan& pl = r.pl;
  const Workspace& ws = r.ws;
  hipStream_t st = r.st;
  const size_t N = pl.N, M2 = pl.M2, BK = pl.BK, WROWS = pl.WROWS;
  BigSection big(r.c, st, BIG_NTT);
  r.sb(ST_QUOTIENT);
  QPointTables wpt;
  wpt.x = ws.wpt;
  wpt.lfirst = ws.wpt + WROWS;
  wpt.llast = ws.wpt + 2 * WROWS;
  for (int h = 0; h < 2; h++)
    for (size_t k0 = 0; k0 < N; k0 += BK) {
      r.tf.for_lde_chunks(ws.tcoef, pl.W, 1 << h, [&](int c0, int cn) {
        fri_extract_window(ws.ldechunk, M2, pl.log_n, h, k0, WROWS, cn, ws.tw + (size_t)c0 * WROWS, st);
      });
      r.tf.for_lde_chunks(ws.acoef, pl.A, 1 << h, [&](int c0, int cn) {
        fri_extract_window(ws.ldechunk, M2, pl.log_n, h, k0, WROWS, cn, ws.aw + (size_t)c0 * WROWS, st);
      });
      quotient_point_tables_window(ws.wpt, ws.wpt + WROWS, ws.wpt + 2 * WROWS, pl.log_n, h, k0, WROWS, st);
      QArgs QA;
      quotient_fill_args(QA, pl.sh, nullptr, nullptr, ws.W, ws.mzt, r.pt, betas, gammas, pl.log_n, ws.qv, ws.qpart);
      quotient_window_args(QA, ws.tw, ws.aw, wpt, ws.qpart, WROWS, BK, k0, h);
      stark_kind(pl.kind).quotient_launch(QA, pl.sh, st);
    }
}

static int stage_quotient(const Run& r, const u64 alphas[2], const u64 betas[2], const u64 gammas[2], u64* cap_out, std::string& err) {
  const ProofPlan& pl = r.pl;
  const Workspace& ws = r.ws;
  const StarkKind& sk = stark_kind(pl.kind);
  hipStream_t st = r.st;
  const size_t N = pl.N;
  {
    std::vector<u64> hW, hmzt;
    const int* mz_e0 = nullptr;
    const int nblk = sk.mz_blocks(&mz_e0);
    quotient_host_tables(pl.K, alphas, mz_e0, nblk, hW, hmzt);
    CHK(hipMemcpyAsync(ws.W, hW.data(), hW.size() * 8, hipMemcpyHostToDevice, st));
    CHK(hipMemcpyAsync(ws.mzt, hmzt.data(), hmzt.size() * 8, hipMemcpyHostToDevice, st));
    CHK(hipStreamSynchronize(st));
  }
  if (pl.stream) {
    quotient_over_windows(r, betas, gammas);
  } else {
    BigSection big(r.c, st, BIG_EXCL);
    r.sb(ST_QUOTIENT);
    QArgs QA;
    quotient_fill_args(QA, pl.sh, ws.tlde, ws.alde, ws.W, ws.mzt, r.pt, betas, gammas, pl.log_n, ws.qv, ws.qpart);
    sk.quotient_launch(QA, pl.sh, st);
  }
  r.tf.quotient_coset_inverse(ws.qv, ws.ab);
  {
    u64 gn = gl_pow(GL_GEN, N);
    u64 inv2 = gl_inv(2), inv2c = gl_inv(gl_mul(2, gn));
    dim3 g((unsigned)((N + 255) / 256), 2);
    k_quotient_chunks<<<g, 256, 0, st>>>(ws.ab, ws.qcoef, N, inv2, inv2c);
  }
  r.se(ST_QUOTIENT);
  r.sb(ST_QUOTIENT_COMMIT);
  r.tf.lde(ws.qcoef, ws.qlde, ProofPlan::NQ);
  merkle_build(ws.qlde, 1, pl.M2, ProofPlan::NQ, pl.log_m2, pl.P.cap_height, ws.qtree, st, r.mmode());
  CHK(hipMemcpyAsync(cap_out, ws.qtree + ws.cap_off, ProofPlan::CAPW * 8, hipMemcpyDeviceToHost, st));
  r.se(ST_QUOTIENT_COMMIT);
  CHK(hipStreamSynchronize(st));
  return BN254S_OK;
}

static int stage_openings(const Run& r, gl2 zeta, gl2 zeta_next, u64* h_part, std::string& err) {
  const ProofPlan& pl = r.pl;
  const Workspace& ws = r.ws;
  hipStream_t st = r.st;
  const int W = pl.W, A = pl.A, NQ = ProofPlan::NQ, NSPL = pl.NSPL;
  const size_t R = pl.R, NH = pl.NH;
  {
    BigSection big(r.c, st, BIG_EXCL);
    r.sb(ST_OPENINGS);
    u64* d_otab = ws.open + pl.n_part();
    fri_opening_tables(pl.log_r, pl.log_s ? gl2_mul(zeta, zeta) : zeta, pl.log_s ? gl2_mul(zeta_next, zeta_next) : zeta_next, d_otab, st);
    fri_openings(ws.tcoef, NH, pl.log_r, W * NSPL, d_otab, ws.open, st);
    fri_openings(ws.acoef, NH, pl.log_r, A * NSPL, d_otab, ws.open + (size_t)W * NSPL * R * 5, st);
    fri_openings(ws.qcoef, NH, pl.log_r, NQ * NSPL, d_otab, ws.open + (size_t)(W + A) * NSPL * R * 5, st);
  }
  CHK(hipMemcpyAsync(h_part, ws.open, pl.n_part() * 8, hipMemcpyDeviceToHost, st));
  r.se(ST_OPENINGS);
  CHK(hipStreamSynchronize(st));
  return BN254S_OK;
}

static std::vector<u64> recombine_openings(const ProofPlan& pl, const u64* h_part, gl2 zeta, gl2 zeta_next) {
  const size_t R = pl.R;
  const int NSPL = pl.NSPL, n_polys = pl.W + pl.A + ProofPlan::NQ;
  std::vector<u64> h_open((size_t)n_polys * 5);
  std::vector<gl2> zp0(R), zp1(R);
  gl2 a = gl2_make(1, 0), b = gl2_make(1, 0);
  const gl2 y0 = pl.log_s ? gl2_mul(zeta, zeta) : zeta, y1 = pl.log_s ? gl2_mul(zeta_next, zeta_next) : zeta_next;
  for (size_t k1 = 0; k1 < R; k1++) {
    zp0[k1] = a;
    zp1[k1] = b;
    a = gl2_mul(a, y0);
    b = gl2_mul(b, y1);
  }
  for (int p = 0; p < n_polys; p++) {
    gl2 v0 = gl2_make(0, 0), v1 = gl2_make(0, 0);
    u64 s1 = 0;
    for (int half = 0; half < NSPL; half++) {
      gl2 e0 = gl2_make(0, 0), e1 = gl2_make(0, 0);
      for (size_t k1 = 0; k1 < R; k1++) {
        const u64* q = &h_part[(((size_t)p * NSPL + half) * R + k1) * 5];
        e0 = gl2_add(e0, gl2_mul(zp0[k1], gl2_make(q[0], q[1])));
        e1 = gl2_add(e1, gl2_mul(zp1[k1], gl2_make(q[2], q[3])));
        s1 = gl_add(s1, q[4]);
      }
      v0 = gl2_add(v0, half ? gl2_mul(zeta, e0) : e0);
      v1 = gl2_add(v1, half ? gl2_mul(zeta_next, e1) : e1);
    }
    u64* o5 = &h_open[(size_t)p * 5];
    o5[0] = v0.c0; o5[1] = v0.c1; o5[2] = v1.c0; o5[3] = v1.c1; o5[4] = s1;
  }
  return h_open;
}

struct Openings {
  const ProofPlan& pl;
  const std::vector<u64>& h_open;
  u64 operator()(int p, int k) const { return h_open[(size_t)p * 5 + k]; }
  int n_ctlz() const { return 2 * pl.sh.n_ctl; }
  u64 ctl_z_first(int i) const { return (*this)(pl.W + pl.sh.n_lookup_cols() + i, 4); }
};

static void observe_openings(Challenger& ch, const Openings& op) {
  const int W = op.pl.W, A = op.pl.A, NQ = ProofPlan::NQ;
  for (int p = 0; p < W + A + NQ; p++) {
    ch.observe(op(p, 0));
    ch.observe(op(p, 1));
  }
  for (int p = 0; p < W + A; p++) {
    ch.observe(op(p, 2));
    ch.observe(op(p, 3));
  }
  for (int i = 0; i < op.n_ctlz(); i++) {
    ch.observe(op.ctl_z_first(i));
    ch.observe(0);
  }
}

struct FriAlphaPowers {
  std::vector<u32> apow;
  gl2 r0, r1, r2;
};
static FriAlphaPowers fri_alpha_powers(const Openings& op, gl2 fri_alpha) {
  const int W = op.pl.W, A = op.pl.A, NQ = ProofPlan::NQ, n_ctlz = op.n_ctlz();
  FriAlphaPowers f;
  f.apow.assign(8 * (size_t)(W + A + NQ), 0);
  gl2 ap = gl2_make(1, 0);
  f.r0 = f.r1 = f.r2 = gl2_make(0, 0);
  for (int p = 0; p < W + A + NQ; p++) {
    fri_weight_record(&f.apow[8 * (size_t)p], ap);
    f.r0 = gl2_add(f.r0, gl2_mul(ap, gl2_make(op(p, 0), op(p, 1))));
    if (p < W + A) f.r1 = gl2_add(f.r1, gl2_mul(ap, gl2_make(op(p, 2), op(p, 3))));
    if (p < n_ctlz) f.r2 = gl2_add(f.r2, gl2_mul_base(ap, op.ctl_z_first(p)));
    ap = gl2_mul(ap, fri_alpha);
  }
  return f;
}

static int stage_fri_combine(const Run& r, const FriAlphaPowers& f, gl2 zeta, gl2 zeta_next, gl2 fri_alpha, std::string& err) {
  const ProofPlan& pl = r.pl;
  const Workspace& ws = r.ws;
  hipStream_t st = r.st;
  CHK(hipMemcpyAsync(ws.apow, f.apow.data(), f.apow.size() * 4, hipMemcpyHostToDevice, st));
  CHK(hipStreamSynchronize(st));
  BigSection big(r.c, st, BIG_EXCL);
  r.sb(ST_FRI);
  fri_combine_coeffs(pl.sh, ws.tcoef, ws.acoef, ws.qcoef, ws.apow, pl.N, ws.comb, st);
  r.tf.lde(ws.comb, ws.comb + (size_t)6 * pl.N, 6);
  fri_combine_final(pl.sh, ws.comb + (size_t)6 * pl.N, r.pt.x, zeta, zeta_next, f.r0, f.r1, f.r2, fri_alpha, pl.M2, ws.fri, st);
  return BN254S_OK;
}

struct FriLayers {
  std::vector<std::vector<u64>> caps;
  std::vector<const u64*> vals, trees;
  const u64* last = nullptr;
  u64 shift = GL_GEN;
  unsigned lm = 0;
};

static int stage_fri_commit(const Run& r, Challenger& ch, FriLayers& fl, std::string& err) {
  const ProofPlan& pl = r.pl;
  hipStream_t st = r.st;
  const int L = pl.L, CAPW = ProofPlan::CAPW;
  fl.caps.assign(L, std::vector<u64>(CAPW));
  fl.vals.resize(L);
  fl.trees.resize(L);
  u64* vals = r.ws.fri;
  u64* ftree = r.ws.fritrees;
  fl.shift = GL_GEN;
  unsigned lm = pl.log_m2;
  const u64 inv16 = gl_inv(16);
  for (int l = 0; l < L; l++) {
    const int lg = (int)lm - 4;
    merkle_build(vals, 32, 1, 32, lg, pl.P.cap_height, ftree, st, r.mmode());
    CHK(hipMemcpyAsync(fl.caps[l].data(), ftree + 4 * merkle_level_offset(lg, lg - pl.P.cap_height), CAPW * 8,
                       hipMemcpyDeviceToHost, st));
    CHK(hipStreamSynchronize(st));
    ch.observe_n(fl.caps[l].data(), CAPW);
    gl2 beta = ch.challenge_ext();
    u64* next = vals + 2 * ((size_t)1 << lm);
    fri_fold(vals, next, lm, fl.shift, beta, inv16, st);
    fl.vals[l] = vals;
    fl.trees[l] = ftree;
    ftree += merkle_tree_digests(lg, pl.P.cap_height) * 4;
    vals = next;
    fl.shift = gl_pow(fl.shift, 16);
    lm -= 4;
  }
  fl.last = vals;
  fl.lm = lm;
  return BN254S_OK;
}

static int fri_final_poly(const std::vector<u64>& h_final, unsigned lm, u64 shift, unsigned rate_bits, std::vector<gl2>& final_poly,
                          std::string& err) {
  const size_t Mf = (size_t)1 << lm;
  final_poly.assign(Mf >> rate_bits, gl2_make(0, 0));
  const u64 w = gl_root_of_unity(lm), winv = gl_inv(w), sinv = gl_inv(shift), minv = gl_inv((u64)Mf);
  for (size_t k = 0; k < Mf; k++) {
    gl2 acc = gl2_make(0, 0);
    u64 wk = gl_pow(winv, k), t = 1;
    for (size_t nn = 0; nn < Mf; nn++) {
      size_t pos = bitrev32((u32)nn, lm);
      acc = gl2_add(acc, gl2_mul_base(gl2_make(h_final[2 * pos], h_final[2 * pos + 1]), t));
      t = gl_mul(t, wk);
    }
    acc = gl2_mul_base(acc, gl_mul(minv, gl_pow(sinv, k)));
    if (k < final_poly.size()) final_poly[k] = acc;
    else if (acc.c0 | acc.c1) {
      err = "FRI final polynomial has non-zero high coefficients";
      return BN254S_E_INTERNAL;
    }
  }
  return BN254S_OK;
}

static int stage_pow(const Run& r, Challenger& ch, u64& pow_witness, std::string& err) {
  const unsigned pow_bits = r.pl.P.pow_bits;
  hipStream_t st = r.st;
  u64 stt[12];
  memcpy(stt, ch.state, sizeof(stt));
  for (int i = 0; i < ch.in_len; i++) stt[i] = ch.in_buf[i];
  const size_t WIN = (size_t)1 << (pow_bits + 1);
  unsigned long long found = ~0ULL;
  for (u64 base = 0; found == ~0ULL; base += WIN) {
    CHK(hipMemsetAsync(r.ws.pow, 0xFF, 8, st));
    fri_pow_launch(stt, ch.in_len, base, pow_bits, WIN, r.ws.pow, st);
    CHK(hipMemcpyAsync(&found, r.ws.pow, 8, hipMemcpyDeviceToHost, st));
    CHK(hipStreamSynchronize(st));
    if (base > ((u64)1 << 40)) {
      err = "proof of work not found";
      return BN254S_E_INTERNAL;
    }
  }
  pow_witness = found;
  ch.observe(pow_witness);
  u64 resp = ch.challenge();
  if (resp >> (64 - pow_bits)) {
    err = "proof of work self-check failed";
    return BN254S_E_INTERNAL;
  }
  return BN254S_OK;
}

static int stage_queries(const Run& r, Challenger& ch, const FriLayers& fl, u64* h_q, std::string& err) {
  const ProofPlan& pl = r.pl;
  const Workspace& ws = r.ws;
  hipStream_t st = r.st;
  const int W = pl.W, A = pl.A, L = pl.L, nq = (int)pl.P.num_queries;
  std::vector<u32> qidx(pl.P.num_queries);
  for (auto& q : qidx) q = (u32)(ch.challenge() % pl.M2);
  CHK(hipMemcpyAsync(ws.qidx, qidx.data(), qidx.size() * 4, hipMemcpyHostToDevice, st));
  if (pl.stream) {
    r.tf.for_lde_chunks(ws.tcoef, W, 3, [&](int c0, int cn) {
      fri_gather_rows(ws.ldechunk, pl.M2, cn, ws.qidx, nq, ws.qrows + (size_t)c0 * nq, st);
    });
    r.tf.for_lde_chunks(ws.acoef, A, 3, [&](int c0, int cn) {
      fri_gather_rows(ws.ldechunk, pl.M2, cn, ws.qidx, nq, ws.qrows + (size_t)(W + c0) * nq, st);
    });
  }
  {
    QueryGatherArgs G;
    G.lde[0] = ws.tlde; G.lde[1] = ws.alde; G.lde[2] = ws.qlde;
    if (pl.stream) {
      G.lde[0] = ws.qrows;
      G.lde[1] = ws.qrows + (size_t)W * pl.P.num_queries;
      G.lde_by_query[0] = G.lde_by_query[1] = 1;
    }
    G.tree[0] = ws.ttree; G.tree[1] = ws.atree; G.tree[2] = ws.qtree;
    G.width[0] = W; G.width[1] = A; G.width[2] = ProofPlan::NQ;
    for (int l = 0; l < L; l++) {
      G.layer_vals[l] = fl.vals[l];
      G.layer_tree[l] = fl.trees[l];
    }
    G.n_layers = L;
    G.log_m2 = pl.log_m2;
    G.cap_height = pl.P.cap_height;
    G.M2 = pl.M2;
    G.indices = ws.qidx;
    G.out = ws.qout;
    G.words_per_query = pl.wpq;
    fri_gather_queries(G, pl.P.num_queries, st);
  }
  int h_err = 0;
  CHK(hipMemcpyAsync(h_q, ws.qout, pl.n_q() * 8, hipMemcpyDeviceToHost, st));
  CHK(hipMemcpyAsync(&h_err, ws.err, 4, hipMemcpyDeviceToHost, st));
  r.se(ST_FRI);
  r.se(ST_TOTAL);
  CHK(hipStreamSynchronize(st));
  CHK(hipGetLastError());
  if (h_err) {
    err = "device self-check failed: " + std::to_string(h_err);
    return h_err;
  }
  return BN254S_OK;
}

struct ProofParts {
  u64 caps[3][64];
  u64 init_state[12];
  std::vector<u64> h_open;
  FriLayers fri;
  std::vector<gl2> final_poly;
  u64 pow_witness = 0;
  const u64* h_q = nullptr;
};

static void assemble_proof(const ProofPlan& pl, const ProofParts& pp, bn254s_proof* pr) {
  const int W = pl.W, A = pl.A, NQ = ProofPlan::NQ, CAPW = ProofPlan::CAPW, L = pl.L;
  const Openings op{pl, pp.h_open};
  const int n_ctlz = op.n_ctlz();
  std::vector<u64>& o = pr->words;
  o.clear();
  o.reserve(3 * CAPW + 4 * (W + A) + n_ctlz + 2 * NQ + L * CAPW + pl.n_q() + 2 * pp.final_poly.size() + 13);
  auto mark = [&](int id) { pr->sec_off[id] = o.size(); };
  for (int t = 0; t < 3; t++) { mark(BN254S_SEC_TRACE_CAP + t); o.insert(o.end(), pp.caps[t], pp.caps[t] + CAPW); }
  mark(BN254S_SEC_LOCAL_VALUES);
  for (int p = 0; p < W; p++) { o.push_back(op(p, 0)); o.push_back(op(p, 1)); }
  mark(BN254S_SEC_NEXT_VALUES);
  for (int p = 0; p < W; p++) { o.push_back(op(p, 2)); o.push_back(op(p, 3)); }
  mark(BN254S_SEC_AUX_POLYS);
  for (int p = W; p < W + A; p++) { o.push_back(op(p, 0)); o.push_back(op(p, 1)); }
  mark(BN254S_SEC_AUX_POLYS_NEXT);
  for (int p = W; p < W + A; p++) { o.push_back(op(p, 2)); o.push_back(op(p, 3)); }
  mark(BN254S_SEC_CTL_ZS_FIRST);
  for (int i = 0; i < n_ctlz; i++) o.push_back(op.ctl_z_first(i));
  mark(BN254S_SEC_QUOTIENT_POLYS);
  for (int p = W + A; p < W + A + NQ; p++) { o.push_back(op(p, 0)); o.push_back(op(p, 1)); }
  mark(BN254S_SEC_FRI_CAPS);
  for (int l = 0; l < L; l++) o.insert(o.end(), pp.fri.caps[l].begin(), pp.fri.caps[l].end());
  mark(BN254S_SEC_QUERY_ROUNDS);
  o.insert(o.end(), pp.h_q, pp.h_q + pl.n_q());
  mark(BN254S_SEC_FINAL_POLY);
  for (auto& cf : pp.final_poly) { o.push_back(cf.c0); o.push_back(cf.c1); }
  mark(BN254S_SEC_POW_WITNESS);
  o.push_back(pp.pow_witness);
  mark(BN254S_SEC_INIT_CHALLENGER_STATE);
  o.insert(o.end(), pp.init_state, pp.init_state + 12);
  mark(BN254S_SEC_COUNT);
  pr->degree_bits = pl.log_n;
}

static int prove_on_slot(bn254s_ctx* c, Slot& sl, int kind, const bn254s_params& P, const u64* scalars, const u64* x,
                         const u64* off, size_t n, bn254s_proof* pr, std::string& err,
                         const std::function<void()>* after_alloc = nullptr) {
  size_t dev_free_b = 0, dev_total_b = 0;
  (void)hipMemGetInfo(&dev_free_b, &dev_total_b);
  ProofPlan pl;
  if (int rc = proof_plan(kind, n, P, dev_total_b, plan_overrides_from_env(), pl, err)) return rc;
  hipStream_t st = sl.st;
  QPointTables pt;
  if (int rc = get_point_tables(c, pl.log_n, pt)) {
    err = "point tables";
    return rc;
  }
  const NttTallTables* TT = nullptr;
  const NttSplitTables* SP = nullptr;
  if (pl.log_r) {
    TT = get_tall_tables(c, pl.log_n - pl.log_s, pl.log_s != 0);
    if (!TT) {
      err = "tall NTT tables";
      return BN254S_E_OOM;
    }
  }
  if (pl.log_s) {
    SP = get_split_tables(c, pl.log_n);
    if (!SP) {
      err = "split NTT tables";
      return BN254S_E_OOM;
    }
  }
  Workspace ws;
  if (int rc = workspace_acquire(sl, pl, ws, err)) return rc;
  if (after_alloc) (*after_alloc)();
  const Transforms tf{c, st, TT, SP, pl, ws.tmp, ws.ldechunk, ws.sponge};
  if (sl.events.empty()) {
    sl.events.resize(2 * ST_COUNT);
    for (auto& e : sl.events) CHK(hipEventCreate(&e));
  }
  const Run r{c, sl, st, pl, ws, tf, pt};
  const int CAPW = ProofPlan::CAPW;
  ProofParts pp;
  Challenger ch;

  r.sb(ST_TOTAL);
  int h_err = 0;
  if (int rc = stage_trace(r, scalars, x, off, pr, &h_err, err)) return rc;
  if (int rc = commit(r, ws.tvals, ws.tcoef, ws.tlde, pl.W, ws.ttree, ST_TRACE_NTT, ST_TRACE_MERKLE, pp.caps[0], err)) return rc;
  if (h_err) {
    err = "trace generation reported device error " + std::to_string(h_err);
    return h_err;
  }
  ch.observe_n(pp.caps[0], CAPW);
  u64 betas[2], gammas[2];
  for (int i = 0; i < 2; i++) {
    betas[i] = ch.challenge();
    gammas[i] = ch.challenge();
  }
  ch.compact(pp.init_state);

  stage_aux(r, betas, gammas);
  if (pl.stream)
    if (int rc = ws.begin_windows(err)) return rc;
  if (int rc = commit(r, ws.avals, ws.acoef, ws.alde, pl.A, ws.atree, ST_AUX_NTT, ST_AUX_MERKLE, pp.caps[1], err)) return rc;
  ch.observe_n(pp.caps[1], CAPW);
  u64 alphas[2] = {ch.challenge(), 0};
  alphas[1] = ch.challenge();

  if (int rc = stage_quotient(r, alphas, betas, gammas, pp.caps[2], err)) return rc;
  ch.observe_n(pp.caps[2], CAPW);
  gl2 zeta = ch.challenge_ext();
  {
    gl2 zp = zeta;
    for (unsigned i = 0; i < pl.log_n; i++) zp = gl2_mul(zp, zp);
    if (gl2_eq(zp, gl2_make(1, 0))) {
      err = "Opening point is in the subgroup.";
      return BN254S_E_TRANSCRIPT;
    }
  }
  const gl2 zeta_next = gl2_mul_base(zeta, gl_root_of_unity(pl.log_n));

  u64* staging = (u64*)sl.pinned;
  if (int rc = stage_openings(r, zeta, zeta_next, staging, err)) return rc;
  pp.h_open = recombine_openings(pl, staging, zeta, zeta_next);
  const Openings op{pl, pp.h_open};
  observe_openings(ch, op);

  const gl2 fri_alpha = ch.challenge_ext();
  if (int rc = stage_fri_combine(r, fri_alpha_powers(op, fri_alpha), zeta, zeta_next, fri_alpha, err)) return rc;
  if (int rc = stage_fri_commit(r, ch, pp.fri, err)) return rc;
  std::vector<u64> h_final((size_t)2 << pp.fri.lm);
  CHK(hipMemcpyAsync(h_final.data(), pp.fri.last, h_final.size() * 8, hipMemcpyDeviceToHost, st));
  CHK(hipStreamSynchronize(st));
  if (int rc = fri_final_poly(h_final, pp.fri.lm, pp.fri.shift, P.rate_bits, pp.final_poly, err)) return rc;
  for (auto& cf : pp.final_poly) {
    ch.observe(cf.c0);
    ch.observe(cf.c1);
  }
  if (int rc = stage_pow(r, ch, pp.pow_witness, err)) return rc;
  pp.h_q = staging;
  if (int rc = stage_queries(r, ch, pp.fri, staging, err)) return rc;

  assemble_proof(pl, pp, pr);
  for (int i = 0; i < ST_COUNT; i++) hipEventElapsedTime(&pr->stage_ms[i], sl.events[2 * i], sl.events[2 * i + 1]);
  return BN254S_OK;
}

extern "C" {

struct bn254s_batch {
  bn254s_ctx* c = nullptr;
  int kind = 0;
  bn254s_params params;
  const u64 *scalars = nullptr, *x = nullptr, *off = nullptr;
  size_t n_total = 0, per_proof = 0, n_proofs = 0;
  bn254s_proof** out = nullptr;
  std::mutex mu;
  std::condition_variable cv;
  size_t remaining = 0;
  int first_rc = 0;
  std::string err;
};

int bn254s_prove_batch_begin(bn254s_ctx* c, int kind, const bn254s_params* params, const uint64_t* scalars, const uint64_t* x,
                             const uint64_t* off, size_t n_total, size_t per_proof, bn254s_proof** proofs_out,
                             bn254s_batch** handle) {
  if (!c || kind < 0 || kind > 2 || !params || !scalars || !x || (kind != KIND_FQ && !off) || !proofs_out || !handle || n_total == 0 ||
      per_proof == 0 || params->struct_size != sizeof(bn254s_params))
    return BN254S_E_INVALID_ARG;
  *handle = nullptr;
  const size_t n_proofs = (n_total + per_proof - 1) / per_proof;
  const size_t PW = stark_kind(kind).point_words;
  for (size_t i = 0; i < n_proofs; i++) proofs_out[i] = nullptr;
  HIP_TRY(c, hipSetDevice(c->device));
  size_t n_slots = 32;
  if (const char* e = getenv("BN254S_SLOTS")) n_slots = std::min((size_t)bn254s_ctx::MAX_SLOTS, (size_t)std::max(1, atoi(e)));
  for (size_t s = 0; s < n_slots; s++)
    if (!c->slot(s)) return BN254S_E_HIP;
  c->workers.start(n_slots, c->device);
  bn254s_batch* B = new bn254s_batch();
  B->c = c;
  B->kind = kind;
  B->params = *params;
  B->scalars = scalars;
  B->x = x;
  B->off = off;
  B->n_total = n_total;
  B->per_proof = per_proof;
  B->n_proofs = n_proofs;
  B->out = proofs_out;
  B->remaining = n_proofs;
  for (size_t i = 0; i < n_proofs; i++)
    c->workers.push([B, i, PW](size_t s) {
      bool skip;
      {
        std::lock_guard<std::mutex> lk(B->mu);
        skip = B->first_rc != 0;
      }
      if (!skip) {
        const size_t b = i * B->per_proof, cnt = std::min(B->per_proof, B->n_total - b);
        bn254s_proof* pr = new bn254s_proof();
        std::string err;
        bn254s_ctx* c = B->c;
        Slot& sl = *c->slot(s);
        auto attempt = [&](const std::function<void()>* after_alloc) {
          err.clear();
          return prove_on_slot(c, sl, B->kind, B->params, B->scalars + 4 * b, B->x + PW * b, B->off ? B->off + PW * b : nullptr, cnt,
                               pr, err, after_alloc);
        };
        int rc = attempt(nullptr);
        WorkPool& wp = c->workers;
        while (rc == BN254S_E_OOM) {
          std::unique_lock<std::mutex> rl(wp.retry_mu);
          const size_t c0 = wp.completions_now();
          wp.for_idle_slots([&](size_t i) {
            if (i < c->n_slots_now()) c->slot(i)->mem.release();
          });
          const bool last = wp.active() <= 1;
          const std::function<void()> unlock = [&]() { rl.unlock(); };
          rc = attempt(&unlock);
          if (rl.owns_lock()) rl.unlock();
          if (rc != BN254S_E_OOM || last) break;
          wp.wait_for_a_completion(c0);
        }
        if (rc != BN254S_OK) {
          hipStreamSynchronize(sl.st);
          delete pr;
          std::lock_guard<std::mutex> lk(B->mu);
          if (B->first_rc == 0) {
            B->first_rc = rc;
            B->err = err;
          }
// ... 187 lines not shown
```

plonky2_bn254_amd/lib.py:

```python
from __future__ import annotations

import ctypes as C
import os
from typing import Optional

import numpy as np

_HERE = os.path.dirname(os.path.abspath(__file__))
LIB_PATH = os.environ.get("BN254S_LIB") or os.path.join(_HERE, "libbn254stark.so")

U64P = C.POINTER(C.c_uint64)


class LibraryMissing(RuntimeError):
    pass


class VerifyError(RuntimeError):
    """bn254s_verify rejected the proof; the message is the reference verifier's error text."""


class Params(C.Structure):
    _fields_ = [(n, C.c_uint32) for n in (
        "struct_size", "security_bits", "num_challenges", "rate_bits", "cap_height", "pow_bits",
        "arity_bits", "final_poly_bits", "num_queries", "min_rows_log2")]


_lib = None


def load_library():
    global _lib
    if _lib is not None:
        return _lib
    if not os.path.exists(LIB_PATH):
        raise LibraryMissing(
            f"{LIB_PATH} not found: build it with `python -c 'import __graft_entry__ as g; g.build()'` "
            "(there is no CPU fallback for the proving path)")
    lib = C.CDLL(LIB_PATH)
    vp = C.c_void_p
    lib.bn254s_abi_version.restype = C.c_int
    lib.bn254s_params_default.argtypes = [C.POINTER(Params)]
    lib.bn254s_ctx_create.argtypes = [C.c_int, C.POINTER(vp)]
    lib.bn254s_ctx_destroy.argtypes = [vp]
    lib.bn254s_ctx_trim.argtypes = [vp]
    lib.bn254s_last_error.argtypes = [vp]
    lib.bn254s_last_error.restype = C.c_char_p
    for name in ("bn254s_prove_g1", "bn254s_prove_g2"):
        getattr(lib, name).argtypes = [vp, C.POINTER(Params), vp, vp, vp, C.c_size_t, C.POINTER(vp)]
    lib.bn254s_prove_fq_exp.argtypes = [vp, C.POINTER(Params), vp, vp, C.c_size_t, C.POINTER(vp)]
    lib.bn254s_generate_trace.argtypes = [vp, C.c_int, vp, vp, vp, C.c_size_t, C.c_uint32, vp, vp]
    lib.bn254s_prove_g1_batch.argtypes = [vp, C.POINTER(Params), vp, vp, vp, C.c_size_t, C.c_size_t, C.POINTER(vp)]
    lib.bn254s_prove_batch.argtypes = [vp, C.c_int, C.POINTER(Params), vp, vp, vp, C.c_size_t, C.c_size_t, C.POINTER(vp)]
    lib.bn254s_prove_batch_begin.argtypes = [vp, C.c_int, C.POINTER(Params), vp, vp, vp, C.c_size_t, C.c_size_t, C.POINTER(vp),
                                             C.POINTER(vp)]
    lib.bn254s_prove_batch_end.argtypes = [vp]
    lib.bn254s_prove_batch_multi.argtypes = [C.POINTER(vp), C.c_size_t, C.c_int, C.POINTER(Params), vp, vp, vp, C.c_size_t,
                                             C.c_size_t, C.POINTER(vp)]
    lib.bn254s_proof_words.argtypes = [vp, C.POINTER(U64P), C.POINTER(C.c_size_t)]
    lib.bn254s_proof_outputs.argtypes = [vp, C.POINTER(U64P), C.POINTER(C.c_size_t)]
    lib.bn254s_proof_degree_bits.argtypes = [vp]
    lib.bn254s_proof_section.argtypes = [vp, C.c_int, C.POINTER(U64P), C.POINTER(C.c_size_t)]
    lib.bn254s_proof_stage_ms.argtypes = [vp, C.POINTER(C.POINTER(C.c_float)), C.POINTER(C.c_size_t)]
    lib.bn254s_stage_name.argtypes = [C.c_size_t]
    lib.bn254s_stage_name.restype = C.c_char_p
    lib.bn254s_proof_free.argtypes = [vp]
    lib.bn254s_proof_serialize.argtypes = [vp, vp, C.c_size_t]
    lib.bn254s_proof_serialize.restype = C.c_size_t
    lib.bn254s_verify.argtypes = [vp, C.c_int, C.POINTER(Params), C.c_uint32, vp, C.c_size_t, vp, vp, vp, vp, C.c_size_t]
    lib.bn254s_verify_host.argtypes = [C.c_int, C.POINTER(Params), C.c_uint32, vp, C.c_size_t, vp, vp, vp, vp, C.c_size_t, C.c_char_p,
                                       C.c_size_t]
    if hasattr(lib, "bn254s_verify_batch"):
        lib.bn254s_verify_batch.argtypes = [vp, C.c_int, C.POINTER(Params), C.c_uint32, vp, C.c_size_t, vp, vp, vp, vp, vp, C.c_size_t,
                                            vp, vp, C.c_size_t]
        lib.bn254s_selftest_verify_front.argtypes = [C.c_int, C.POINTER(Params), C.c_uint32, vp, C.c_size_t, vp, C.c_size_t]
        lib.bn254s_selftest_query_round.argtypes = [vp, C.c_int, C.POINTER(Params), C.c_uint32, vp, C.c_size_t, vp, C.c_size_t,
                                                    C.c_size_t, vp]
        lib.bn254s_selftest_verify_batch_ms.argtypes = [vp, vp]
        lib.bn254s_selftest_query_text.argtypes = [C.c_int, C.c_int]
        lib.bn254s_selftest_query_text.restype = C.c_char_p
    lib.bn254s_map_to_g2.argtypes = [vp, C.POINTER(Params), vp, vp, C.c_size_t, vp, vp, vp, C.POINTER(vp), C.POINTER(vp)]
    lib.bn254s_hash_to_fq2.argtypes = [vp, C.c_size_t, vp]
    lib.bn254s_g1_msm_chain.argtypes = [vp, vp, vp, vp, C.c_size_t, vp, vp]
    lib.bn254s_g1_msm.argtypes = [vp, C.POINTER(Params), vp, vp, vp, C.c_size_t, C.c_size_t, vp, vp, C.POINTER(vp)]
    lib.bn254s_g2_msm_chain.argtypes = [vp, vp, vp, vp, C.c_size_t, vp, vp]
    lib.bn254s_g2_msm.argtypes = [vp, C.POINTER(Params), vp, vp, vp, C.c_size_t, C.c_size_t, vp, vp, C.POINTER(vp)]
    lib.bn254s_g1_recover_from_x_batch.argtypes = [vp, vp, C.c_size_t, vp, vp, vp]
    lib.bn254s_g1_recover_from_x.argtypes = [vp, C.POINTER(Params), vp, C.c_size_t, C.c_size_t, vp, vp, vp, C.POINTER(vp)]
    lib.bn254s_g2_recover_from_x_batch.argtypes = [vp, vp, vp, C.c_size_t, vp, vp, vp]
    lib.bn254s_g2_recover_from_x.argtypes = [vp, C.POINTER(Params), vp, vp, C.c_size_t, C.c_size_t, vp, vp, vp, C.POINTER(vp)]
    lib.bn254s_g2_subgroup_check_batch.argtypes = [vp, vp, C.c_size_t, vp]
    lib.bn254s_g2_subgroup_check.argtypes = [vp, C.POINTER(Params), vp, vp, C.c_size_t, C.c_size_t, vp, vp, C.POINTER(vp)]
    lib.bn254s_g2_clear_cofactor_batch.argtypes = [vp, vp, C.c_size_t, vp, vp]
    lib.bn254s_g2_clear_cofactor.argtypes = [vp, C.POINTER(Params), vp, vp, C.c_size_t, C.c_size_t, vp, vp, vp, C.POINTER(vp)]
    lib.bn254s_map_to_g2_batch.argtypes = [vp, vp, C.c_size_t, vp]
    lib.bn254s_hash_to_g2_batch.argtypes = [vp, vp, C.c_size_t, C.c_size_t, vp]
    lib.bn254s_job_outputs_batch.argtypes = [vp, C.c_int, vp, vp, vp, C.c_size_t, vp, vp]
    lib.bn254s_job_outputs.argtypes = [vp, C.c_int, C.POINTER(Params), vp, vp, vp, C.c_size_t, C.c_size_t, vp, C.POINTER(vp)]
    lib.bn254s_hash_to_fq2_batch.argtypes = [vp, vp, C.c_size_t, C.c_size_t, vp]
    if hasattr(lib, "bn254s_map_to_g1"):
        lib.bn254s_hash_to_fq.argtypes = [vp, C.c_size_t, vp]
        lib.bn254s_hash_to_fq_batch.argtypes = [vp, vp, C.c_size_t, C.c_size_t, vp]
        lib.bn254s_map_to_g1_batch.argtypes = [vp, vp, C.c_size_t, vp, vp, vp]
        lib.bn254s_hash_to_g1_batch.argtypes = [vp, vp, C.c_size_t, C.c_size_t, vp]
        lib.bn254s_map_to_g1.argtypes = [vp, C.POINTER(Params), vp, C.c_size_t, C.c_size_t, vp, vp, vp, C.POINTER(vp)]
    lib.bn254s_ctl_values.argtypes = [C.c_int, vp, vp, vp, vp, C.c_size_t, vp, vp]
    lib.bn254s_commit_values.argtypes = [vp, vp, C.c_size_t, vp, vp, vp]
    lib.bn254s_bench_ntt.argtypes = [vp, C.c_size_t, C.c_int, C.POINTER(C.c_float)]
    lib.bn254s_bench_ntt_clock.argtypes = [vp, C.c_size_t, C.c_int, C.POINTER(C.c_float), C.POINTER(C.c_float), C.POINTER(C.c_float)]
    lib.bn254s_bench_issue.argtypes = [vp, C.POINTER(C.c_float), C.POINTER(C.c_float)]
    lib.bn254s_poseidon_permute.argtypes = [vp, vp, C.c_size_t]
    lib.bn254s_selftest_field.argtypes = [vp, vp, vp, C.c_size_t, vp]
    lib.bn254s_selftest_poseidon.argtypes = [vp, C.c_int, vp, C.c_size_t]
    lib.bn254s_selftest_leaf_hash.argtypes = [vp, vp, C.c_size_t, C.c_int, C.c_int, C.c_int, vp]
    lib.bn254s_selftest_fq_inv.argtypes = [vp, vp, C.c_size_t, vp]
    lib.bn254s_selftest_fq.argtypes = [vp, C.c_int, vp, C.c_size_t, vp]
    if hasattr(lib, "bn254s_selftest_logup"):
        lib.bn254s_selftest_logup.argtypes = [vp, vp, C.c_size_t, C.c_int, C.c_int, C.c_int, C.c_int, C.c_int, vp, vp]
    if hasattr(lib, "bn254s_selftest_fri_fold"):
        lib.bn254s_selftest_acc.argtypes = [vp, vp, vp, C.c_size_t, C.c_size_t, vp]
        lib.bn254s_selftest_openings.argtypes = [vp, vp, C.c_int, C.c_int, vp, vp, vp]
        lib.bn254s_selftest_fri_combine.argtypes = [vp, C.c_int, C.c_int, C.c_int, C.c_int, C.c_size_t, vp, vp, vp, vp]
        lib.bn254s_selftest_fri_fold.argtypes = [vp, vp, C.c_int, C.c_uint64, vp, vp]
        lib.bn254s_selftest_fri_rows.argtypes = [vp, vp, C.c_int, C.c_int, C.c_int, C.c_size_t, C.c_size_t, vp, C.c_int, vp, vp]
    if hasattr(lib, "bn254s_selftest_proof_plan"):
        lib.bn254s_selftest_proof_plan.argtypes = [C.c_int, C.c_size_t, C.POINTER(Params), C.c_uint64, C.c_int, C.c_int, C.c_int,
                                                   C.c_int, vp, C.c_char_p, C.c_size_t]
    lib.bn254s_bench_copy.argtypes = [vp, C.c_size_t, C.c_int]
    lib.bn254s_bench_leafhash.argtypes = [vp, C.c_size_t, C.c_int, C.c_int, C.POINTER(C.c_float)]
    lib.bn254s_g1_generate_trace.argtypes = [vp, vp, vp, vp, C.c_size_t, C.c_uint32, vp, vp]
    _lib = lib
    return lib


def default_params() -> Params:
    p = Params()
    load_library().bn254s_params_default(C.byref(p))
    return p


def _ptr(a: Optional[np.ndarray]):
    if a is None:
        return None
    assert a.dtype == np.uint64 and a.flags["C_CONTIGUOUS"]
    return a.ctypes.data_as(C.c_void_p)


def _slots(n_jobs, per_proof):
    return (C.c_void_p * ((n_jobs + per_proof - 1) // per_proof))()


def _proofs(lib, slots):
    return [Proof(lib, C.c_void_p(h)) for h in slots]


class Proof:

    _stage_names = None

    def __init__(self, lib, handle):
        self._lib, self._h = lib, handle
        self._words = self._outputs = None
        self.degree_bits = lib.bn254s_proof_degree_bits(handle)
        ms, k = C.POINTER(C.c_float)(), C.c_size_t()
        lib.bn254s_proof_stage_ms(handle, C.byref(ms), C.byref(k))
        if Proof._stage_names is None or len(Proof._stage_names) != k.value:
            Proof._stage_names = [lib.bn254s_stage_name(i).decode() for i in range(k.value)]
        self.stage_ms = dict(zip(Proof._stage_names, ms[:k.value]))

    def _fetch(self, fn, what):
        if not self._h:
            raise RuntimeError(f"Proof.{what}: the proof was closed before its {what} were read")
        data, n = U64P(), C.c_size_t()
        rc = fn(self._h, C.byref(data), C.byref(n))
        if rc != 0:
            raise RuntimeError(f"bn254s_proof_{what} failed with {rc}")
        return data, n.value

    @property
    def words(self) -> np.ndarray:
        if self._words is None:
            data, n = self._fetch(self._lib.bn254s_proof_words, "words")
            self._words = np.ctypeslib.as_array(data, shape=(n,)).copy()
        return self._words

    @property
    def outputs(self) -> np.ndarray:
        if self._outputs is None:
            data, n = self._fetch(self._lib.bn254s_proof_outputs, "outputs")
            self._outputs = np.ctypeslib.as_array(data, shape=(n,)).copy() if n else np.zeros(0, np.uint64)
        return self._outputs

    def caps(self) -> np.ndarray:
        if self._words is not None:
            return self._words[:192].copy()
        data, n = self._fetch(self._lib.bn254s_proof_words, "words")
        assert n >= 192
        return np.ctypeslib.as_array(data, shape=(192,)).copy()

    SECTIONS = ("trace_cap", "auxiliary_polys_cap", "quotient_polys_cap", "local_values", "next_values", "auxiliary_polys",
                "auxiliary_polys_next", "ctl_zs_first", "quotient_polys", "commit_phase_merkle_caps", "query_round_proofs",
                "final_poly", "pow_witness", "init_challenger_state")

    def section(self, name: str) -> np.ndarray:
        data, n = U64P(), C.c_size_t()
        rc = self._lib.bn254s_proof_section(self._h, self.SECTIONS.index(name), C.byref(data), C.byref(n))
        if rc != 0:
            raise RuntimeError(f"bn254s_proof_section({name}) failed with {rc}")
        return np.ctypeslib.as_array(data, shape=(n.value,)).copy() if n.value else np.zeros(0, np.uint64)

    def serialize(self) -> bytes:
        need = self._lib.bn254s_proof_serialize(self._h, None, 0)
        buf = C.create_string_buffer(need)
        assert self._lib.bn254s_proof_serialize(self._h, buf, need) == need
        return buf.raw

    def close(self):
        if self._h:
            try:
                self.words, self.outputs
            finally:
                self._lib.bn254s_proof_free(self._h)
                self._h = None

    def __del__(self):
        if getattr(self, "_h", None):
            self._lib.bn254s_proof_free(self._h)
            self._h = None


class Context:

    def __init__(self, device: int = 0):
        self._h = None
        self._lib = load_library()
        h = C.c_void_p()
        rc = self._lib.bn254s_ctx_create(device, C.byref(h))
        if rc != 0:
            raise RuntimeError(f"bn254s_ctx_create(device={device}) failed with {rc} (is a GPU visible?)")
        self._h = h
        self.device = device

    def close(self):
        if self._h:
            self._lib.bn254s_ctx_destroy(self._h)
            self._h = None

    def __del__(self):
        self.close()

    def trim(self):
        self._check(self._lib.bn254s_ctx_trim(self._h), "bn254s_ctx_trim")

    def _check(self, rc, what):
        if rc != 0:
            raise RuntimeError(f"{what} failed with {rc}: {self._lib.bn254s_last_error(self._h).decode()}")

    def prove_g1(self, scalars, x, offset, params: Optional[Params] = None) -> Proof:
        params = params or default_params()
        n = scalars.shape[0]
        out = C.c_void_p()
        self._check(self._lib.bn254s_prove_g1(self._h, C.byref(params), _ptr(scalars), _ptr(x), _ptr(offset), n,
                                              C.byref(out)), "bn254s_prove_g1")
        return Proof(self._lib, out)

    def prove_g2(self, scalars, x, offset, params: Optional[Params] = None) -> Proof:
        params = params or default_params()
        out = C.c_void_p()
        self._check(self._lib.bn254s_prove_g2(self._h, C.byref(params), _ptr(scalars), _ptr(x), _ptr(offset),
                                              scalars.shape[0], C.byref(out)), "bn254s_prove_g2")
        return Proof(self._lib, out)

    def prove_fq_exp(self, scalars, x, params: Optional[Params] = None) -> Proof:
        params = params or default_params()
        out = C.c_void_p()
        self._check(self._lib.bn254s_prove_fq_exp(self._h, C.byref(params), _ptr(scalars), _ptr(x), scalars.shape[0],
                                                  C.byref(out)), "bn254s_prove_fq_exp")
        return Proof(self._lib, out)

    def prove_g1_batch(self, scalars, x, offset, per_proof=128, params: Optional[Params] = None, keep=True):
        params = params or default_params()
        n = scalars.shape[0]
        outs = _slots(n, per_proof)
        self._check(self._lib.bn254s_prove_g1_batch(self._h, C.byref(params), _ptr(scalars), _ptr(x), _ptr(offset), n,
                                                    per_proof, outs), "bn254s_prove_g1_batch")
        return _proofs(self._lib, outs)

    def prove_batch(self, kind, scalars, x, offset=None, per_proof=128, params: Optional[Params] = None):
        params = params or default_params()
        n = scalars.shape[0]
        outs = _slots(n, per_proof)
        self._check(self._lib.bn254s_prove_batch(self._h, kind, C.byref(params), _ptr(scalars), _ptr(x), _ptr(offset), n,
                                                 per_proof, outs), "bn254s_prove_batch")
        return _proofs(self._lib, outs)

    def prove_batch_begin(self, kind, scalars, x, offset=None, per_proof=128, params: Optional[Params] = None):
        return BatchInFlight(self, kind, scalars, x, offset, per_proof, params or default_params())

    def verify(self, kind, words, degree_bits, scalars, x, offset, outputs, params: Optional[Params] = None):
        params = params or default_params()
        words = np.ascontiguousarray(words, dtype=np.uint64)
        outputs = np.ascontiguousarray(outputs, dtype=np.uint64)
        rc = self._lib.bn254s_verify(self._h, kind, C.byref(params), degree_bits, _ptr(words), words.size, _ptr(scalars), _ptr(x),
                                     _ptr(offset), _ptr(outputs), scalars.shape[0])
        if rc == -8:
            raise VerifyError(self._lib.bn254s_last_error(self._h).decode())
        self._check(rc, "bn254s_verify")

    def verify_batch(self, kind, proofs, scalars, x, offset, n_jobs=None, params: Optional[Params] = None, degree_bits=None):
        return _verify_batch(self._lib, self._h, kind, proofs, scalars, x, offset, n_jobs, params, degree_bits)

    def verify_batch_ms(self) -> dict:
        ms = (C.c_float * 5)()
        self._check(self._lib.bn254s_selftest_verify_batch_ms(self._h, ms), "bn254s_selftest_verify_batch_ms")
        return dict(zip(("front", "upload", "k_vb_merkle", "k_vb_fri", "ctl"), (float(v) for v in ms)))

    def query_round(self, kind, words, degree_bits, records, chunk_proofs=0, params: Optional[Params] = None) -> np.ndarray:
        return query_round(kind, words, degree_bits, records, chunk_proofs, params, _ctx=self)

    def map_to_g2(self, u, offsets, params: Optional[Params] = None):
        params = params or default_params()
        n = u.shape[0]
        pts = np.zeros((n, 16), np.uint64)
        fq_jobs = np.zeros((2 * n, 8), np.uint64)
        g2_jobs = np.zeros((n, 20), np.uint64)
        pf, pg = _slots(2 * n, 128), _slots(n, 128)
        self._check(self._lib.bn254s_map_to_g2(self._h, C.byref(params), _ptr(u), _ptr(offsets), n, _ptr(pts), _ptr(fq_jobs),
                                               _ptr(g2_jobs), pf, pg), "bn254s_map_to_g2")
        return pts, fq_jobs, g2_jobs, _proofs(self._lib, pf), _proofs(self._lib, pg)

    def _msm_chain(self, fn, w, scalars, x, offset):
        scalars, x, offset = (np.ascontiguousarray(a, dtype=np.uint64) for a in (scalars, x, offset))
        n = scalars.shape[0]
        offs = np.zeros((n + 1, w), np.uint64)
        res = np.zeros(w, np.uint64)
        self._check(getattr(self._lib, fn)(self._h, _ptr(scalars), _ptr(x), _ptr(offset), n, _ptr(offs), _ptr(res)), fn)
        return offs, res

    def _msm(self, fn, w, scalars, x, offset, per_proof, params):
        params = params or default_params()
        scalars, x, offset = (np.ascontiguousarray(a, dtype=np.uint64) for a in (scalars, x, offset))
        n = scalars.shape[0]
        offs = np.zeros((n + 1, w), np.uint64)
        res = np.zeros(w, np.uint64)
        outs = _slots(n, per_proof)
        self._check(getattr(self._lib, fn)(self._h, C.byref(params), _ptr(scalars), _ptr(x), _ptr(offset), n, per_proof, _ptr(res),
                                           _ptr(offs), outs), fn)
        return res, offs, _proofs(self._lib, outs)

    def g1_msm_chain(self, scalars, x, offset):
        return self._msm_chain("bn254s_g1_msm_chain", 8, scalars, x, offset)

    def g1_msm(self, scalars, x, offset, per_proof=128, params: Optional[Params] = None):
        return self._msm("bn254s_g1_msm", 8, scalars, x, offset, per_proof, params)

    def g2_msm_chain(self, scalars, x, offset):
        return self._msm_chain("bn254s_g2_msm_chain", 16, scalars, x, offset)

    def g2_msm(self, scalars, x, offset, per_proof=128, params: Optional[Params] = None):
        return self._msm("bn254s_g2_msm", 16, scalars, x, offset, per_proof, params)

    def g1_recover_from_x_batch(self, xs):
        xs = np.ascontiguousarray(xs, dtype=np.uint64)
        n = xs.shape[0]
        pts, flags, jobs = np.zeros((n, 8), np.uint64), np.zeros(n, np.uint8), np.zeros((n, 8), np.uint64)
        self._check(self._lib.bn254s_g1_recover_from_x_batch(self._h, _ptr(xs), n, _ptr(pts), flags.ctypes.data_as(C.c_void_p),
                                                             _ptr(jobs)), "bn254s_g1_recover_from_x_batch")
        return pts, flags, jobs

    def g1_recover_from_x(self, xs, per_proof=128, params: Optional[Params] = None):
        params = params or default_params()
        xs = np.ascontiguousarray(xs, dtype=np.uint64)
        n = xs.shape[0]
        pts, flags, jobs = np.zeros((n, 8), np.uint64), np.zeros(n, np.uint8), np.zeros((n, 8), np.uint64)
        outs = _slots(n, per_proof)
        self._check(self._lib.bn254s_g1_recover_from_x(self._h, C.byref(params), _ptr(xs), n, per_proof, _ptr(pts),
                                                       flags.ctypes.data_as(C.c_void_p), _ptr(jobs), outs), "bn254s_g1_recover_from_x")
        return pts, flags, jobs, _proofs(self._lib, outs)

    @staticmethod
    def _sgns(sgns, n):
        if sgns is None:
            return None, None
        sgns = np.ascontiguousarray(sgns, dtype=np.uint8).reshape(-1)
        if sgns.shape[0] != n:
            raise ValueError(f"{sgns.shape[0]} sgns for {n} xs")
        return sgns, sgns.ctypes.data_as(C.c_void_p)

    def g2_recover_from_x_batch(self, xs, sgns=None):
        xs = np.ascontiguousarray(xs, dtype=np.uint64)
        n = xs.shape[0]
        sgns, sp = self._sgns(sgns, n)
        pts, flags, jobs = np.zeros((n, 16), np.uint64), np.zeros(n, np.uint8), np.zeros((n, 8), np.uint64)
        self._check(self._lib.bn254s_g2_recover_from_x_batch(self._h, _ptr(xs), sp, n, _ptr(pts), flags.ctypes.data_as(C.c_void_p),
                                                             _ptr(jobs)), "bn254s_g2_recover_from_x_batch")
        return pts, flags, jobs

    def g2_recover_from_x(self, xs, sgns=None, per_proof=128, params: Optional[Params] = None):
        params = params or default_params()
        xs = np.ascontiguousarray(xs, dtype=np.uint64)
        n = xs.shape[0]
        sgns, sp = self._sgns(sgns, n)
        pts, flags, jobs = np.zeros((n, 16), np.uint64), np.zeros(n, np.uint8), np.zeros((n, 8), np.uint64)
        outs = _slots(n, per_proof)
        self._check(self._lib.bn254s_g2_recover_from_x(self._h, C.byref(params), _ptr(xs), sp, n, per_proof, _ptr(pts),
                                                       flags.ctypes.data_as(C.c_void_p), _ptr(jobs), outs), "bn254s_g2_recover_from_x")
        return pts, flags, jobs, _proofs(self._lib, outs)

    def g2_subgroup_check_batch(self, points):
# ... 277 lines not shown
        self._check(self._lib.bn254s_poseidon_permute(self._h, _ptr(st), st.shape[0]), "bn254s_poseidon_permute")
        return st

    def generate_trace(self, kind, scalars, x, offset=None, min_rows_log2=16):
        width, pw = {0: (781, 8), 1: (1295, 16), 2: (427, 4)}[kind]
        n = scalars.shape[0]
        rows = max(1 << min_rows_log2, 512 * n)
        rows = 1 << (rows - 1).bit_length()
        trace = np.zeros((width, rows), np.uint64)
        outs = np.zeros((n, pw), np.uint64)
        self._check(self._lib.bn254s_generate_trace(self._h, kind, _ptr(scalars), _ptr(x), _ptr(offset), n, min_rows_log2,
                                                    _ptr(trace), _ptr(outs)), "bn254s_generate_trace")
        return trace, outs

    def g1_generate_trace(self, scalars, x, offset, min_rows_log2=16, width=781):
        n = scalars.shape[0]
        rows = max(1 << min_rows_log2, 512 * n)
        rows = 1 << (rows - 1).bit_length()
        trace = np.zeros((width, rows), np.uint64)
        outs = np.zeros((n, 8), np.uint64)
        self._check(self._lib.bn254s_g1_generate_trace(self._h, _ptr(scalars), _ptr(x), _ptr(offset), n, min_rows_log2,
                                                       _ptr(trace), _ptr(outs)), "bn254s_g1_generate_trace")
        return trace, outs


def verify_host(kind, words, degree_bits, scalars, x, offset, outputs, params: Optional[Params] = None):
    lib = load_library()
    params = params or default_params()
    words = np.ascontiguousarray(words, dtype=np.uint64)
    outputs = np.ascontiguousarray(outputs, dtype=np.uint64)
    buf = C.create_string_buffer(256)
    rc = lib.bn254s_verify_host(kind, C.byref(params), degree_bits, _ptr(words), words.size, _ptr(scalars), _ptr(x), _ptr(offset),
                                _ptr(outputs), scalars.shape[0], buf, 256)
    if rc == -8:
        raise VerifyError(buf.value.decode())
    if rc != 0:
        raise RuntimeError(f"bn254s_verify_host failed with {rc}: {buf.value.decode()}")


_POINT_WORDS = (8, 16, 4)
VERIFY_RECORD_HEAD = 34


def proof_words(kind, degree_bits, params: Optional[Params] = None) -> int:
    params = params or default_params()
    plan = proof_plan(kind, 1, 0)
    w, a = plan["W"], plan["A"]
    log_m2 = degree_bits + params.rate_bits
    path = log_m2 - params.cap_height
    wpq = w + a + 4 + 12 * path
    d, bits, layers = degree_bits, log_m2, 0
    while d > params.final_poly_bits and d + params.rate_bits - params.arity_bits >= params.cap_height:
        d -= params.arity_bits
        bits -= params.arity_bits
        layers += 1
        wpq += (2 << params.arity_bits) + 4 * (bits - params.cap_height)
    return 192 + 4 * w + 4 * a + 4 + 8 + 64 * layers + params.num_queries * wpq + (2 << d) + 1 + 12


def _word_arrays(word_list):
    arrs = [np.ascontiguousarray(w, dtype=np.uint64).reshape(-1) for w in word_list]
    table = (C.c_void_p * len(arrs))(*[a.ctypes.data for a in arrs])
    return arrs, table


def _verify_batch(lib, handle, kind, proofs, scalars, x, offset, n_jobs, params, degree_bits):
    params = params or default_params()
    pw = _POINT_WORDS[kind]
    words, outs = [], []
    for pr in proofs:
        if isinstance(pr, (tuple, list)):
            w, o = pr
        else:
            w, o = pr.words, pr.outputs
            degree_bits = pr.degree_bits if degree_bits is None else degree_bits
        words.append(np.ascontiguousarray(w, dtype=np.uint64).reshape(-1))
        outs.append(np.ascontiguousarray(o, dtype=np.uint64).reshape(-1))
    n = len(words)
    if n == 0:
        raise ValueError("verify_batch: no proofs")
    if degree_bits is None:
        sizes = {proof_words(kind, d, params): d for d in range(7, 31)}
        degree_bits = next((sizes[w.size] for w in words if w.size in sizes), None)
        if degree_bits is None:
            raise ValueError("verify_batch: cannot tell degree_bits from the proof sizes, pass it")
    if n_jobs is None:
        n_jobs = [o.size // pw for o in outs]
    n_jobs = [int(k) for k in n_jobs]
    lo = np.concatenate(([0], np.cumsum(n_jobs)))
    scalars = np.ascontiguousarray(scalars, dtype=np.uint64).reshape(-1, 4)
    x = np.ascontiguousarray(x, dtype=np.uint64).reshape(-1, pw)
    offset = None if offset is None else np.ascontiguousarray(offset, dtype=np.uint64).reshape(-1, pw)
    verdicts = [None] * n
    groups = {}
    for i, w in enumerate(words):
        groups.setdefault(w.size, []).append(i)
    for n_words, idx in groups.items():
        rows = np.concatenate([np.arange(lo[i], lo[i + 1]) for i in idx]).astype(np.int64)
        whole = len(groups) == 1
        s_, x_ = (scalars, x) if whole else (np.ascontiguousarray(scalars[rows]), np.ascontiguousarray(x[rows]))
        o_ = offset if whole or offset is None else np.ascontiguousarray(offset[rows])
        outputs = np.ascontiguousarray(np.concatenate([outs[i] for i in idx]))
        arrs, table = _word_arrays([words[i] for i in idx])
        m = len(idx)
        nj = (C.c_size_t * m)(*[n_jobs[i] for i in idx])
        status = np.zeros(m, dtype=np.int32)
        stride = 128
        err = C.create_string_buffer(m * stride)
        rc = lib.bn254s_verify_batch(handle, kind, C.byref(params), degree_bits, table, n_words, _ptr(s_), _ptr(x_), _ptr(o_),
                                     _ptr(outputs), nj, m, status.ctypes.data_as(C.c_void_p), err, stride)
        if rc not in (0, -8):
            why = lib.bn254s_last_error(handle).decode() if handle else ""
            raise RuntimeError(f"bn254s_verify_batch failed with {rc}: {why}")
        for k, i in enumerate(idx):
            if status[k] != 0:
                verdicts[i] = err.raw[k * stride:(k + 1) * stride].split(b"\0", 1)[0].decode()
    return verdicts


def verify_batch_host(kind, proofs, scalars, x, offset, n_jobs=None, params: Optional[Params] = None, degree_bits=None):
    return _verify_batch(load_library(), None, kind, proofs, scalars, x, offset, n_jobs, params, degree_bits)


def verify_front(kind, words, degree_bits, params: Optional[Params] = None):
    lib = load_library()
    params = params or default_params()
    words = np.ascontiguousarray(words, dtype=np.uint64)
    rec = np.zeros(VERIFY_RECORD_HEAD + params.num_queries, dtype=np.uint64)
    rc = lib.bn254s_selftest_verify_front(kind, C.byref(params), degree_bits, _ptr(words), words.size, _ptr(rec), rec.size)
    return rc, rec


def query_round(kind, words, degree_bits, records, chunk_proofs=0, params: Optional[Params] = None, _ctx=None) -> np.ndarray:
    lib = load_library()
    params = params or default_params()
    arrs, table = _word_arrays(words)
    records = np.ascontiguousarray(records, dtype=np.uint64).reshape(len(arrs), -1)
    if records.shape[1] != VERIFY_RECORD_HEAD + params.num_queries:
        raise ValueError("query_round: records of the wrong length")
    codes = np.full((len(arrs), params.num_queries), -1, dtype=np.int32)
    rc = lib.bn254s_selftest_query_round(_ctx._h if _ctx is not None else None, kind, C.byref(params), degree_bits, table,
                                         arrs[0].size, _ptr(records), len(arrs), chunk_proofs, codes.ctypes.data_as(C.c_void_p))
    if rc != 0:
        why = lib.bn254s_last_error(_ctx._h).decode() if _ctx is not None else ""
        raise RuntimeError(f"bn254s_selftest_query_round failed with {rc}: {why}")
    return codes


def query_text(n_layers, code):
    t = load_library().bn254s_selftest_query_text(n_layers, code)
    return None if t is None else t.decode()


PLAN_BUFFERS = ("in", "tvals", "tcoef", "hist", "tmp", "ldechunk", "sponge", "comb", "tlde", "trees", "avals", "acoef", "alde",
                "scratch", "quot", "tabs", "open", "fri", "fritrees", "qout", "win")
_PLAN_HEAD = ("kind", "n", "W", "A", "K", "point_words", "N", "log_n", "log_s", "log_r", "R", "NH", "NSPL", "stream", "lowmem",
              "log_bk", "BK", "WROWS", "L")
_PLAN_TAIL = ("wpq", "tree_words", "fri_words", "fri_tree_words", "in_words")


def proof_plan(kind, n, dev_total_bytes, force_split=False, force_lowmem=False, force_stream=False, stream_win_log=None,
               params: Optional[Params] = None) -> dict:
    lib = load_library()
    params = params or default_params()
    out = np.zeros(54, np.uint64)
    buf = C.create_string_buffer(256)
    rc = lib.bn254s_selftest_proof_plan(kind, n, C.byref(params), dev_total_bytes, int(force_split), int(force_lowmem), int(force_stream),
                                        -1 if stream_win_log is None else stream_win_log, _ptr(out), buf, 256)
    if rc != 0:
        raise RuntimeError(f"bn254s_selftest_proof_plan failed with {rc}: {buf.value.decode()}")
    v = [int(w) for w in out]
    plan = dict(zip(_PLAN_HEAD, v[:19]))
    plan["arities"] = v[19:19 + plan["L"]]
    plan.update(zip(_PLAN_TAIL, v[27:32]))
    plan["words"] = dict(zip(PLAN_BUFFERS, v[32:53]))
    plan["pinned_bytes"] = v[53]
    return plan


def _proof_slices(tag, proofs, n, per_proof, w):
    if len(proofs) != (n + per_proof - 1) // per_proof:
        raise VerifyError(f"{tag}: {len(proofs)} proofs for {n} jobs of {per_proof} per proof")

    def walk():
        for k, pr in enumerate(proofs):
            lo, hi = k * per_proof, min(n, (k + 1) * per_proof)
            outs = np.asarray(pr.outputs, dtype=np.uint64).reshape(-1, w)
            if outs.shape[0] != hi - lo:
                raise VerifyError(f"{tag}: proof {k} has {outs.shape[0]} outputs for jobs {lo}..{hi - 1}")
            yield k, pr, lo, hi, outs
    return walk()


def _verify_slice(tag, kind, k, pr, lo, hi, scalars, x, offset, ctx, params):
    s_, x_, o_ = (None if a is None else np.ascontiguousarray(a[lo:hi]) for a in (scalars, x, offset))
    try:
        if ctx is not None:
            ctx.verify(kind, pr.words, pr.degree_bits, s_, x_, o_, pr.outputs, params)
        else:
            verify_host(kind, pr.words, pr.degree_bits, s_, x_, o_, pr.outputs, params)
    except VerifyError as e:
        raise VerifyError(f"{tag}: proof {k} (jobs {lo}..{hi - 1}) rejected: {e}") from None


def _check_legendre(tag, p, k, lo, hi, outs, flags, note=lambda j: ("", "")):
    from tools import synth

    for j in range(lo, hi):
        leg = synth.words_to_int(outs[j - lo])
        if leg not in (1, p - 1):
            raise VerifyError(f"{tag}: output {j} of proof {k}{note(j)[0]} is neither 1 nor p - 1")
        if (leg == 1) != bool(flags[j]):
            raise VerifyError(f"{tag}: flag {j}{note(j)[1]} is {int(flags[j])}, the proven Legendre symbol of job {j} is "
                              f"{'1' if leg == 1 else 'p - 1'}")


def _verify_msm(tag, kind, w, pt, neg, add, scalars, x, R, result, offsets, proofs, per_proof, ctx, params):
    scalars, x, R, result, offsets = (np.ascontiguousarray(a, dtype=np.uint64) for a in (scalars, x, R, result, offsets))
    n = scalars.shape[0]
    offsets = offsets.reshape(-1, w)
    if x.shape != (n, w) or offsets.shape != (n + 1, w) or R.size != w or result.size != w:
        raise VerifyError(f"{tag}: shapes: scalars {scalars.shape}, x {x.shape}, offsets {offsets.shape}, R {R.shape}, result {result.shape}")
    slices = _proof_slices(tag, proofs, n, per_proof, w)
    if not np.array_equal(offsets[0], R.reshape(w)):
        raise VerifyError(f"{tag}: offsets[0] != R")
    for i, pr, lo, hi, outs in slices:
        bad = np.nonzero(np.any(outs != offsets[lo + 1:hi + 1], axis=1))[0]
        if bad.size:
            j = lo + int(bad[0])
            raise VerifyError(f"{tag}: output {j} of proof {i} != offsets[{j + 1}] (link s_{j} x_{j} + offset_{j})")
    try:
        want = add(pt(offsets[n]), neg(pt(R.reshape(w))))
    except ValueError:
        raise VerifyError(f"{tag}: offsets[n] == R, the result would be the point at infinity") from None
    if pt(result.reshape(w)) != want:
        raise VerifyError(f"{tag}: result != offsets[n] - R")
    for i, pr, lo, hi, _ in _proof_slices(tag, proofs, n, per_proof, w):
        _verify_slice(tag, kind, i, pr, lo, hi, scalars, x, offsets, ctx, params)


def verify_g1_msm(scalars, x, R, result, offsets, proofs, per_proof, ctx: Optional[Context] = None, params: Optional[Params] = None):
    from tools import synth

    def pt(w):
        return (synth.words_to_int(w[:4]), synth.words_to_int(w[4:]))

    _verify_msm("g1_msm", 0, 8, pt, lambda p: (p[0], (-p[1]) % synth.P), synth.g1_add, scalars, x, R, result, offsets, proofs,
                per_proof, ctx, params)


def verify_g2_msm(scalars, x, R, result, offsets, proofs, per_proof, ctx: Optional[Context] = None, params: Optional[Params] = None):
    from tools import synth

    def neg(p):
        return (p[0], ((-p[1][0]) % synth.P, (-p[1][1]) % synth.P))

    _verify_msm("g2_msm", 1, 16, synth.g2_from_words, neg, synth.g2_add, scalars, x, R, result, offsets, proofs, per_proof, ctx,
                params)


def verify_g1_recover(xs, points, flags, fq_jobs, proofs, per_proof, ctx: Optional[Context] = None, params: Optional[Params] = None):
    from tools import synth

    tag, p = "g1_recover", synth.P
    xs, points, fq_jobs = (np.ascontiguousarray(a, dtype=np.uint64) for a in (xs, points, fq_jobs))
    flags = np.asarray(flags).reshape(-1)
    n = xs.shape[0]
    if xs.shape != (n, 4) or points.shape != (n, 8) or fq_jobs.shape != (n, 8) or flags.shape != (n,):
        raise VerifyError(f"{tag}: shapes: xs {xs.shape}, points {points.shape}, flags {flags.shape}, fq_jobs {fq_jobs.shape}")
    slices = _proof_slices(tag, proofs, n, per_proof, 4)
    g = []
    for i in range(n):
        x = synth.words_to_int(xs[i])
        if x >= p:
            raise VerifyError(f"{tag}: x_{i} is not below p")
        g.append((x * x * x + 3) % p)
        if synth.words_to_int(fq_jobs[i, :4]) != (p - 1) // 2:
            raise VerifyError(f"{tag}: scalar of job {i} != (p - 1)/2")
        if synth.words_to_int(fq_jobs[i, 4:]) != g[i]:
            raise VerifyError(f"{tag}: x of job {i} != x_{i}^3 + 3")
    for k, pr, lo, hi, outs in slices:
        _verify_slice(tag, 2, k, pr, lo, hi, fq_jobs[:, :4], fq_jobs[:, 4:], None, ctx, params)
        _check_legendre(tag, p, k, lo, hi, outs, flags)
    for i in range(n):
        px, py = synth.words_to_int(points[i, :4]), synth.words_to_int(points[i, 4:])
        if px != synth.words_to_int(xs[i]):
            raise VerifyError(f"{tag}: point {i} does not carry x_{i}")
        if flags[i]:
            if py >= p or py & 1 or py * py % p != g[i]:
                raise VerifyError(f"{tag}: y of point {i} is not the even root of x_{i}^3 + 3 below p")
        elif py != 0:
            raise VerifyError(f"{tag}: point {i} is not (x_{i}, 0) although its flag is clear")


def verify_map_to_g1(u, points, sq_flags, fq_jobs, proofs, per_proof, ctx: Optional[Context] = None, params: Optional[Params] = None):
    from tools import map_to_g1_ref as ref
    from tools import synth

    tag, p = "map_to_g1", synth.P
    u, points, fq_jobs = (np.ascontiguousarray(a, dtype=np.uint64) for a in (u, points, fq_jobs))
    sq_flags = np.asarray(sq_flags).reshape(-1)
    n = u.shape[0]
    if u.shape != (n, 4) or points.shape != (n, 8) or fq_jobs.shape != (2 * n, 8) or sq_flags.shape != (2 * n,):
        raise VerifyError(f"{tag}: shapes: u {u.shape}, points {points.shape}, sq_flags {sq_flags.shape}, fq_jobs {fq_jobs.shape}")
    slices = _proof_slices(tag, proofs, 2 * n, per_proof, 4)
    us = []
# ... 195 lines not shown
```

Baseline: 91.02 proofs/s.

## Hand off NTT scheduler slot early via events and rework big-section admission

Moves the GPU big-section admission scheduler into a BigSched struct that makes explicit admit/handoff decisions, replacing the condition-variable broadcast polling. Adds an early-release path for commit NTT sections: once the event recorded before the last NTT kernel completes, the slot goes to the next waiter, which makes its stream wait on the done event. The aim is to shorten idle gaps between host synchronisation and the next admitted section. It also adds optional scheduler logging and stats. The cost is more host-side event synchronisation and the risk of overlapping NTT work beyond the intended cap.

```diff
diff --git a/include/bn254_stark.h b/include/bn254_stark.h
--- a/include/bn254_stark.h
+++ b/include/bn254_stark.h
@@ -206,6 +206,11 @@
 #define BN254S_PLAN_WORDS 54
 int bn254s_selftest_proof_plan(int kind, size_t n, const bn254s_params* params, uint64_t dev_total_bytes, int force_split,
                                int force_lowmem, int force_stream, int stream_win_log, uint64_t* out, char* err, size_t err_len);
+#define BN254S_SCHED_LOG_WORDS 8
+size_t bn254s_sched_log(bn254s_ctx* ctx, double* out, size_t cap_entries);
+int bn254s_sched_stats(bn254s_ctx* ctx, uint64_t* out);
+int bn254s_selftest_big_sched(const int* policy, const int* script, size_t n_steps, uint64_t* admissions, size_t cap_admissions,
+                              size_t* n_admissions, uint32_t* admitted_after);
 int bn254s_generate_trace(bn254s_ctx* ctx, int kind, const uint64_t* scalars, const uint64_t* x, const uint64_t* offset,
                           size_t n, uint32_t min_rows_log2, uint64_t* trace_out, uint64_t* outputs);
 int bn254s_g1_generate_trace(bn254s_ctx* ctx, const uint64_t* scalars, const uint64_t* x, const uint64_t* offset,
diff --git a/plonky2_bn254_amd/__init__.py b/plonky2_bn254_amd/__init__.py
--- a/plonky2_bn254_amd/__init__.py
+++ b/plonky2_bn254_amd/__init__.py
@@ -2,4 +2,4 @@
 
 _os.environ.setdefault("GPU_MAX_HW_QUEUES", "16")
 
-from .lib import Context, Proof, load_library, LibraryMissing, VerifyError, default_params, proof_plan, proof_words, prove_batch_multi, query_round, query_text, verify_g1_msm, verify_g1_recover, verify_g2_clear_cofactor, verify_g2_msm, verify_g2_recover, verify_batch_host, verify_front, verify_g2_subgroup, verify_host, verify_job_outputs, verify_map_to_g1
+from .lib import Context, Proof, load_library, LibraryMissing, VerifyError, big_sched_script, default_params, proof_plan, proof_words, prove_batch_multi, query_round, query_text, verify_g1_msm, verify_g1_recover, verify_g2_clear_cofactor, verify_g2_msm, verify_g2_recover, verify_batch_host, verify_front, verify_g2_subgroup, verify_host, verify_job_outputs, verify_map_to_g1
diff --git a/plonky2_bn254_amd/csrc/big_sched.h b/plonky2_bn254_amd/csrc/big_sched.h
--- /dev/null
+++ b/plonky2_bn254_amd/csrc/big_sched.h
@@ -0,0 +1,117 @@
+#pragma once
+#include <condition_variable>
+#include <deque>
+#include <mutex>
+#include <vector>
+
+enum { BIG_NTT = 0, BIG_EXCL = 1, BIG_HASH = 2, BIG_HASH_PART = 3, BIG_CLASSES = 4 };
+
+struct BigSched {
+  int cap = 12, cost[BIG_CLASSES] = {12, 2, 4, 2};
+  bool fifo = true;
+  int convoy = 4;
+
+  struct Waiter {
+    unsigned long id = 0;
+    int cls = 0;
+    bool admitted = false;
+    void* after = nullptr;
+    unsigned long after_id = 0;
+    int used_at = 0;
+    std::condition_variable cv;
+  };
+  struct Stats {
+    unsigned long sections[BIG_CLASSES] = {0, 0, 0, 0}, early_releases = 0, behind_event = 0;
+    int max_used = 0;
+  };
+
+  std::mutex mu;
+  std::deque<Waiter*> q;
+  unsigned long next_id = 0;
+  int used = 0, convoy_run = 0;
+  bool after_ntt = false;
+  void* pending = nullptr;
+  unsigned long pending_id = 0;
+  Stats stats;
+  std::vector<unsigned long>* order = nullptr;
+
+  int decide(bool* in_order) const {
+    *in_order = true;
+    if (q.empty()) return -1;
+    if (!fifo) {
+      for (size_t i = 0; i < q.size(); i++)
+        if (used + cost[q[i]->cls] <= cap) return (int)i;
+      return -1;
+    }
+    const Waiter* head = q.front();
+    if (after_ntt && used == 0 && head->cls != BIG_NTT && convoy_run < convoy)
+      for (size_t i = 1; i < q.size(); i++)
+        if (q[i]->cls == BIG_NTT) {
+          *in_order = false;
+          return (int)i;
+        }
+    return used + cost[head->cls] <= cap ? 0 : -1;
+  }
+  void admit_locked() {
+    for (;;) {
+      bool in_order;
+      const int i = decide(&in_order);
+      if (i < 0) return;
+      Waiter* w = q[i];
+      q.erase(q.begin() + i);
+      if (fifo) convoy_run = in_order ? 0 : convoy_run + 1;
+      after_ntt = false;
+      used += cost[w->cls];
+      w->used_at = used;
+      w->after = pending;
+      w->after_id = pending_id;
+      stats.sections[w->cls]++;
+      if (pending) stats.behind_event++;
+      if (used > stats.max_used) stats.max_used = used;
+      if (order) order->push_back(w->id);
+      w->admitted = true;
+      w->cv.notify_one();
+    }
+  }
+  void arrive_locked(Waiter* w, int cls) {
+    w->cls = cls;
+    w->id = next_id++;
+    w->admitted = false;
+    q.push_back(w);
+    admit_locked();
+  }
+  void arrive(Waiter* w, int cls) {
+    std::lock_guard<std::mutex> lk(mu);
+    arrive_locked(w, cls);
+  }
+  void acquire(Waiter* w, int cls) {
+    std::unique_lock<std::mutex> lk(mu);
+    arrive_locked(w, cls);
+    w->cv.wait(lk, [&] { return w->admitted; });
+  }
+  void release_locked(const Waiter* w) {
+    used -= cost[w->cls];
+    after_ntt = w->cls == BIG_NTT && used == 0;
+  }
+  void release(const Waiter* w) {
+    std::lock_guard<std::mutex> lk(mu);
+    release_locked(w);
+    admit_locked();
+  }
+  void release_early(const Waiter* w, void* token) {
+    std::lock_guard<std::mutex> lk(mu);
+    release_locked(w);
+    pending = token;
+    pending_id = w->id;
+    stats.early_releases++;
+    admit_locked();
+  }
+  void finish_early(const Waiter* w) {
+    std::lock_guard<std::mutex> lk(mu);
+    if (pending && pending_id == w->id) pending = nullptr;
+  }
+  Stats stats_now() {
+    std::lock_guard<std::mutex> lk(mu);
+    return stats;
+  }
+};
diff --git a/plonky2_bn254_amd/csrc/capi.hip b/plonky2_bn254_amd/csrc/capi.hip
--- a/plonky2_bn254_amd/csrc/capi.hip
+++ b/plonky2_bn254_amd/csrc/capi.hip
@@ -50,22 +50,32 @@
   c->device = device_id;
   merkle_set_throughput_mode(getenv("BN254S_COOP_MAX_NODES") ? atol(getenv("BN254S_COOP_MAX_NODES")) : -1,
                              getenv("BN254S_MERKLE_LEVEL_ASM") ? atoi(getenv("BN254S_MERKLE_LEVEL_ASM")) : -1);
-  if (const char* e = getenv("BN254S_BIG_CAP")) c->big_cap = std::max(1, atoi(e));
-  if (const char* e = getenv("BN254S_SCHED_FIFO")) c->big_fifo = atoi(e) != 0;
-  if (const char* e = getenv("BN254S_NTT_CONVOY")) c->big_convoy = std::max(0, atoi(e));
+  BigSched& big = c->big;
+  if (const char* e = getenv("BN254S_BIG_CAP")) big.cap = std::max(1, atoi(e));
+  if (const char* e = getenv("BN254S_SCHED_FIFO")) big.fifo = atoi(e) != 0;
+  if (const char* e = getenv("BN254S_NTT_CONVOY")) big.convoy = std::max(0, atoi(e));
   if (const char* e = getenv("BN254S_HASH_SPLIT")) c->hash_split = std::min(8, std::max(1, atoi(e)));
-  c->big_cost[BIG_NTT] = c->big_cap;
+  if (const char* e = getenv("BN254S_SCHED_HANDOFF")) c->sched_handoff = atoi(e) != 0;
+  big.cost[BIG_NTT] = big.cap;
   const char* cost_env[3] = {"BN254S_BIG_COST_NTT", "BN254S_BIG_COST_EXCL", "BN254S_BIG_COST_HASH"};
   for (int k = 0; k < 3; k++) {
-    if (const char* e = getenv(cost_env[k])) c->big_cost[k] = atoi(e);
-    c->big_cost[k] = std::min(c->big_cap, std::max(0, c->big_cost[k]));
-  }
-  c->big_cost[BIG_HASH_PART] = std::max(1, c->big_cost[BIG_HASH] / c->hash_split);
+    if (const char* e = getenv(cost_env[k])) big.cost[k] = atoi(e);
+    big.cost[k] = std::min(big.cap, std::max(0, big.cost[k]));
+  }
+  big.cost[BIG_HASH_PART] = std::max(1, big.cost[BIG_HASH] / c->hash_split);
   if (hipStreamCreateWithFlags(&c->stream, hipStreamNonBlocking) != hipSuccess) {
     delete c;
     return BN254S_E_HIP;
   }
+  if (const char* e = getenv("BN254S_SCHED_LOG"))
+    if (atoi(e) != 0 && !c->sched_log.enable(c->stream)) {
+      c->sched_log.destroy();
+      hipStreamDestroy(c->stream);
+      delete c;
+      return BN254S_E_HIP;
+    }
   if (ntt_tables_init(&c->ntt) != 0) {
+    c->sched_log.destroy();
     delete c;
     return BN254S_E_OOM;
   }
@@ -100,9 +110,12 @@
     s->mem.release();
     if (s->pinned) hipHostFree(s->pinned);
     for (auto& e : s->events) hipEventDestroy(e);
+    if (s->ntt_tail) hipEventDestroy(s->ntt_tail);
+    if (s->ntt_done) hipEventDestroy(s->ntt_done);
     hipStreamDestroy(s->st);
     delete s;
   }
+  c->sched_log.destroy();
   for (auto& kv : c->tall) {
     ntt_tall_tables_free(kv.second);
     delete kv.second;
@@ -141,6 +154,81 @@
 }
 
 const char* bn254s_last_error(const bn254s_ctx* c) { return c ? c->err.c_str() : "null context"; }
+
+size_t bn254s_sched_log(bn254s_ctx* c, double* out, size_t cap) {
+  if (!c || !c->sched_log.on || (!out && cap)) return 0;
+  SchedLog& L = c->sched_log;
+  std::lock_guard<std::mutex> lk(L.mu);
+  const size_t first = L.n > SchedLog::CAP ? L.n - SchedLog::CAP : 0;
+  size_t k = 0;
+  for (size_t i = first; i < L.n && k < cap; i++) {
+    const SchedLog::Entry& en = L.ring[i % SchedLog::CAP];
+    if (!en.closed) continue;
+    float b = 0, e = 0;
+    if (hipEventElapsedTime(&b, L.epoch, en.b) != hipSuccess || hipEventElapsedTime(&e, L.epoch, en.e) != hipSuccess) {
+      (void)hipGetLastError();
+      continue;
+    }
+    double* o = out + BN254S_SCHED_LOG_WORDS * k++;
+    o[0] = en.cls;
+    o[1] = en.slot;
+    o[2] = b;
+    o[3] = e;
+    o[4] = (double)en.id;
+    o[5] = en.behind ? (double)en.after_id : -1.0;
+    o[6] = en.used_at;
+    o[7] = 0;
+  }
+  return k;
+}
+
+int bn254s_sched_stats(bn254s_ctx* c, uint64_t* out) {
+  if (!c || !out) return BN254S_E_INVALID_ARG;
+  const BigSched::Stats s = c->big.stats_now();
+  for (int k = 0; k < BIG_CLASSES; k++) out[k] = s.sections[k];
+  out[4] = s.early_releases;
+  out[5] = s.behind_event;
+  out[6] = (uint64_t)s.max_used;
+  out[7] = c->sched_handoff ? 1 : 0;
+  return BN254S_OK;
+}
+
+int bn254s_selftest_big_sched(const int* policy, const int* script, size_t n_steps, uint64_t* admissions, size_t cap_admissions,
+                              size_t* n_admissions, uint32_t* admitted_after) {
+  if (!policy || (!script && n_steps) || !n_admissions || (!admissions && cap_admissions)) return BN254S_E_INVALID_ARG;
+  BigSched S;
+  S.cap = policy[0];
+  for (int k = 0; k < BIG_CLASSES; k++) S.cost[k] = policy[1 + k];
+  S.fifo = policy[5] != 0;
+  S.convoy = policy[6];
+  std::vector<unsigned long> order;
+  S.order = &order;
+  std::deque<BigSched::Waiter> w;
+  std::vector<char> state;
+  static int token;
+  for (size_t i = 0; i < n_steps; i++) {
+    const int op = script[2 * i], arg = script[2 * i + 1];
+    if (op == 0) {
+      if (arg < 0 || arg >= BIG_CLASSES) return BN254S_E_INVALID_ARG;
+      w.emplace_back();
+      state.push_back(0);
+      S.arrive(&w.back(), arg);
+    } else {
+      if (arg < 0 || (size_t)arg >= w.size() || !w[arg].admitted) return BN254S_E_INVALID_ARG;
+      if (op == 1 && state[arg] == 0) S.release(&w[arg]), state[arg] = 2;
+      else if (op == 2 && state[arg] == 0 && w[arg].cls == BIG_NTT) S.release_early(&w[arg], &token), state[arg] = 1;
+      else if (op == 3 && state[arg] == 1) S.finish_early(&w[arg]), state[arg] = 2;
+      else return BN254S_E_INVALID_ARG;
+    }
+    if (admitted_after) admitted_after[i] = (uint32_t)order.size();
+  }
+  *n_admissions = order.size();
+  for (size_t k = 0; k < order.size() && k < cap_admissions; k++) {
+    admissions[2 * k] = order[k];
+    admissions[2 * k + 1] = w[order[k]].after ? 1 + w[order[k]].after_id : 0;
+  }
+  return BN254S_OK;
+}
 
 int bn254s_commit_values(bn254s_ctx* c, const uint64_t* values, size_t ncols, uint64_t* coeffs, uint64_t* lde,
                          uint64_t* cap) {
diff --git a/plonky2_bn254_amd/csrc/ctx.h b/plonky2_bn254_amd/csrc/ctx.h
--- a/plonky2_bn254_amd/csrc/ctx.h
+++ b/plonky2_bn254_amd/csrc/ctx.h
@@ -14,6 +14,7 @@
 #include "../../include/bn254_stark.h"
 #include "gl_dev.h"
 #include "ntt.h"
+#include "big_sched.h"
 
 struct BufPool {
   std::map<std::string, std::pair<void*, size_t>> pool;
@@ -54,9 +55,59 @@
   void* pinned = nullptr;
   size_t pinned_bytes = 0;
   std::vector<hipEvent_t> events;
-};
-
-enum { BIG_NTT = 0, BIG_EXCL = 1, BIG_HASH = 2, BIG_HASH_PART = 3 };
+  int index = -1;
+  hipEvent_t ntt_tail = nullptr, ntt_done = nullptr;
+};
+
+struct SchedLog {
+  static constexpr size_t CAP = 512;
+  struct Entry {
+    int cls = 0, slot = -1, used_at = 0;
+    unsigned long id = 0, after_id = 0;
+    bool behind = false, closed = false;
+    hipEvent_t b = nullptr, e = nullptr;
+  };
+  bool on = false;
+  hipEvent_t epoch = nullptr;
+  std::mutex mu;
+  std::vector<Entry> ring;
+  size_t n = 0;
+  bool enable(hipStream_t st) {
+    ring.resize(CAP);
+    if (hipEventCreate(&epoch) != hipSuccess) return false;
+    for (Entry& en : ring)
+      if (hipEventCreate(&en.b) != hipSuccess || hipEventCreate(&en.e) != hipSuccess) return false;
+    if (hipEventRecord(epoch, st) != hipSuccess || hipEventSynchronize(epoch) != hipSuccess) return false;
+    on = true;
+    return true;
+  }
+  Entry* open(const BigSched::Waiter& w, int slot) {
+    std::lock_guard<std::mutex> lk(mu);
+    Entry* en = &ring[n++ % CAP];
+    en->cls = w.cls;
+    en->slot = slot;
+    en->used_at = w.used_at;
+    en->id = w.id;
+    en->after_id = w.after_id;
+    en->behind = w.after != nullptr;
+    en->closed = false;
+    return en;
+  }
+  void close(Entry* en) {
+    std::lock_guard<std::mutex> lk(mu);
+    en->closed = true;
+  }
+  void destroy() {
+    for (Entry& en : ring) {
+      if (en.b) hipEventDestroy(en.b);
+      if (en.e) hipEventDestroy(en.e);
+    }
+    ring.clear();
+    if (epoch) hipEventDestroy(epoch);
+    epoch = nullptr;
+    on = false;
+  }
+};
 
 struct WorkPool {
   std::mutex mu;
@@ -167,64 +218,10 @@
   WorkPool workers;
   std::map<unsigned, NttTallTables*> tall;
   std::map<unsigned, NttSplitTables*> split;
-  std::mutex big_mu;
-  std::condition_variable big_cv;
-  int big_cap = 12, big_cost[4] = {12, 2, 4, 2}, big_used = 0;
+  BigSched big;
   int hash_split = 1;
-  bool big_fifo = true;
-  struct BigWaiter {
-    unsigned long id;
-    int cls;
-  };
-  std::deque<BigWaiter> big_q;
-  unsigned long big_next_id = 0;
-  int big_convoy = 4, big_convoy_run = 0;
-  bool big_last_was_ntt = false;
-  void big_lock(int cls) {
-    std::unique_lock<std::mutex> lk(big_mu);
-    if (big_fifo) {
-      const unsigned long my = big_next_id++;
-      big_q.push_back({my, cls});
-      big_cv.wait(lk, [&] {
-        if (big_q.front().id == my) {
-          if (big_used + big_cost[cls] > big_cap) return false;
-          if (big_last_was_ntt && cls != BIG_NTT && big_convoy_run < big_convoy)
-            for (const BigWaiter& w : big_q)
-              if (w.cls == BIG_NTT) return false;
-          return true;
-        }
-        if (cls != BIG_NTT || !big_last_was_ntt || big_used != 0 || big_convoy_run >= big_convoy) return false;
-        if (big_q.front().cls == BIG_NTT) return false;
-        for (const BigWaiter& w : big_q) {
-          if (w.cls == BIG_NTT) return w.id == my;
-        }
-        return false;
-      });
-      const bool in_order = big_q.front().id == my;
-      for (auto it = big_q.begin(); it != big_q.end(); ++it)
-        if (it->id == my) {
-          big_q.erase(it);
-          break;
-        }
-      if (in_order) big_convoy_run = 0;
-      else big_convoy_run++;
-      big_last_was_ntt = false;
-      big_used += big_cost[cls];
-      lk.unlock();
-      big_cv.notify_all();
-      return;
-    }
-    big_cv.wait(lk, [&] { return big_used + big_cost[cls] <= big_cap; });
-    big_used += big_cost[cls];
-  }
-  void big_unlock(int cls) {
-    {
-      std::lock_guard<std::mutex> lk(big_mu);
-      big_used -= big_cost[cls];
-      big_last_was_ntt = cls == BIG_NTT && big_used == 0;
-    }
-    big_cv.notify_all();
-  }
+  bool sched_handoff = true;
+  SchedLog sched_log;
   static constexpr size_t MAX_SLOTS = 64;
   std::mutex slots_mu, err_mu;
   float vb_ms[5] = {0, 0, 0, 0, 0};
@@ -246,6 +243,7 @@
         delete s;
         return nullptr;
       }
+      s->index = (int)slots.size();
       slots.push_back(s);
     }
     return slots[i];
diff --git a/plonky2_bn254_amd/csrc/ntt.h b/plonky2_bn254_amd/csrc/ntt.h
--- a/plonky2_bn254_amd/csrc/ntt.h
+++ b/plonky2_bn254_amd/csrc/ntt.h
@@ -18,7 +18,8 @@
 void ntt_inverse(const NttTables* T, const u64* values, u64* coeffs, u64* tmp, int ncols, hipStream_t s);
 void ntt_coset_inverse(const NttTables* T, int h, const u64* values, u64* coeffs, u64* tmp, int ncols, hipStream_t s);
 void ntt_lde(const NttTables* T, const u64* coeffs, u64* lde, u64* tmp, int ncols, hipStream_t s);
-void ntt_inverse_lde(const NttTables* T, const u64* values, u64* coeffs, u64* lde, u64* tmp, u64* tmp2, int ncols, hipStream_t s);
+void ntt_inverse_lde(const NttTables* T, const u64* values, u64* coeffs, u64* lde, u64* tmp, u64* tmp2, int ncols, hipStream_t s,
+                     hipEvent_t before_last = nullptr);
 void ntt_coset_forward_natural(const NttTables* T, int h, const u64* coeffs, u64* values, u64* tmp, int ncols, hipStream_t s);
 
 struct NttTallTables {
diff --git a/plonky2_bn254_amd/csrc/ntt.hip b/plonky2_bn254_amd/csrc/ntt.hip
--- a/plonky2_bn254_amd/csrc/ntt.hip
+++ b/plonky2_bn254_amd/csrc/ntt.hip
@@ -298,7 +298,8 @@
     k_ntt_pass2<false, true><<<grid, block, 0, s>>>(tmp, NTT_N, lde + (size_t)h * NTT_N, 2 * NTT_N, nullptr, 1, T->tw256_fwd, 0);
   }
 }
-void ntt_inverse_lde(const NttTables* T, const u64* values, u64* coeffs, u64* lde, u64* tmp, u64* tmp2, int ncols, hipStream_t s) {
+void ntt_inverse_lde(const NttTables* T, const u64* values, u64* coeffs, u64* lde, u64* tmp, u64* tmp2, int ncols, hipStream_t s,
+                     hipEvent_t before_last) {
   dim3 grid(16, ncols), block(256);
   u64* y0 = tmp2;
   u64* y1 = tmp2 + (size_t)ncols * NTT_N;
@@ -306,6 +307,7 @@
   k_ntt_intt2_lde1<8><<<grid, block, 0, s>>>(tmp, NTT_N, coeffs, NTT_N, y0, y1, NTT_N, T->tw256_inv, T->coset_pow[0],
                                           T->coset_pow[1], T->twmat_fwd, T->tw256_fwd, 0);
   k_ntt_pass2<false, true><<<grid, block, 0, s>>>(y0, NTT_N, lde, 2 * NTT_N, nullptr, 1, T->tw256_fwd, 0);
+  if (before_last) (void)hipEventRecord(before_last, s);
   k_ntt_pass2<false, true><<<grid, block, 0, s>>>(y1, NTT_N, lde + NTT_N, 2 * NTT_N, nullptr, 1, T->tw256_fwd, 0);
 }
 void ntt_coset_forward_natural(const NttTables* T, int h, const u64* coeffs, u64* values, u64* tmp, int ncols, hipStream_t s) {
diff --git a/plonky2_bn254_amd/csrc/prover.hip b/plonky2_bn254_amd/csrc/prover.hip
--- a/plonky2_bn254_amd/csrc/prover.hip
+++ b/plonky2_bn254_amd/csrc/prover.hip
@@ -120,17 +120,6 @@
   return t;
 }
 
-struct BigSection {
-  bn254s_ctx* c;
-  hipStream_t st;
-  int cls;
-  BigSection(bn254s_ctx* c_, hipStream_t st_, int cls_) : c(c_), st(st_), cls(cls_) { c->big_lock(cls); }
-  ~BigSection() {
-    hipStreamSynchronize(st);
-    c->big_unlock(cls);
-  }
-};
-
 static int get_point_tables(bn254s_ctx* c, unsigned log_n, QPointTables& pt) {
   static std::mutex mu;
   std::lock_guard<std::mutex> lk(mu);
@@ -278,7 +267,7 @@
   u64* eo() const { return tmp; }
   u64* ntmp() const { return tmp + (size_t)CH * 2 * pl.N; }
 
-  void commit_ntt(const u64* vals, u64* coef, u64* lde, int nc) const {
+  void commit_ntt(const u64* vals, u64* coef, u64* lde, int nc, hipEvent_t before_last = nullptr) const {
     const size_t N = pl.N, M2 = pl.M2;
     if (pl.log_s) {
       for (int c0 = 0; c0 < nc; c0 += CH) {
@@ -295,7 +284,7 @@
     } else if (pl.log_r) {
       ntt_inverse_lde_tall(&c->ntt, TT, vals, coef, lde, tmp, nc, st);
     } else {
-      ntt_inverse_lde(&c->ntt, vals, coef, lde, tmp, tmp + (size_t)nc * N, nc, st);
+      ntt_inverse_lde(&c->ntt, vals, coef, lde, tmp, tmp + (size_t)nc * N, nc, st, before_last);
     }
   }
   void lde(const u64* coef, u64* out, int nc) const {
@@ -362,6 +351,39 @@
   int mmode() const { return c->workers.in_flight.load(std::memory_order_relaxed) >= 4 ? MERKLE_THROUGHPUT : MERKLE_LATENCY; }
 };
 
+struct BigSection {
+  bn254s_ctx* c;
+  hipStream_t st;
+  BigSched::Waiter w;
+  SchedLog::Entry* log = nullptr;
+  bool released = false;
+  BigSection(const Run& r, int cls) : c(r.c), st(r.st) {
+    c->big.acquire(&w, cls);
+    if (w.after) hipStreamWaitEvent(st, (hipEvent_t)w.after, 0);
+    if (c->sched_log.on) {
+      log = c->sched_log.open(w, r.sl.index);
+      hipEventRecord(log->b, st);
+    }
+  }
+  void release_behind(hipEvent_t tail, hipEvent_t done) {
+    if (log) hipEventRecord(log->e, st);
+    hipEventRecord(done, st);
+    hipEventSynchronize(tail);
+    c->big.release_early(&w, done);
+    hipEventSynchronize(done);
+    c->big.finish_early(&w);
+    if (log) c->sched_log.close(log);
+    released = true;
+  }
+  ~BigSection() {
+    if (released) return;
+    if (log) hipEventRecord(log->e, st);
+    hipStreamSynchronize(st);
+    c->big.release(&w);
+    if (log) c->sched_log.close(log);
+  }
+};
+
 static int upload_and_generate(const StarkKind& sk, const u64* scalars, const u64* x, const u64* off, size_t n, u64* d_in, u64* d_trace,
                                size_t N, u64* d_scr, u64* d_outs, int* d_err, hipStream_t st, bool with_range, std::string& err) {
   const size_t PW = sk.point_words;
@@ -389,7 +411,7 @@
   if (int rc = upload_and_generate(stark_kind(pl.kind), scalars, x, off, pl.n, ws.in, ws.tvals, pl.N, ws.scr, d_outs, ws.err, st, false, err))
     return rc;
   {
-    BigSection big(r.c, st, BIG_EXCL);
+    BigSection big(r, BIG_EXCL);
     launch_range_columns(ws.tvals, pl.N, sh.rc_begin, sh.rc_end, sh.freq_col, sh.table_col, (u32*)ws.hist, ws.err, st);
   }
   pr->outputs.resize(pl.n * (size_t)pl.PW);
@@ -404,14 +426,14 @@
   const size_t M2 = r.pl.M2;
   const int S = r.pl.log_n == 16 ? c->hash_split : 1;
   if (S <= 1) {
-    BigSection big(c, r.st, BIG_HASH);
+    BigSection big(r, BIG_HASH);
     r.sb(stage);
     merkle_leaves(lde, 1, M2, width, r.pl.log_m2, tree, r.st);
     return;
   }
   const size_t cnt = M2 / S;
   for (int k = 0; k < S; k++) {
-    BigSection big(c, r.st, BIG_HASH_PART);
+    BigSection big(r, BIG_HASH_PART);
     if (k == 0) r.sb(stage);
     merkle_leaves_range(lde, 1, M2, width, (size_t)k * cnt, cnt, tree, r.st);
   }
@@ -422,17 +444,19 @@
   const ProofPlan& pl = r.pl;
   hipStream_t st = r.st;
   if (pl.stream) {
-    BigSection big(r.c, st, BIG_NTT);
+    BigSection big(r, BIG_NTT);
     r.sb(ntt_stage);
     r.tf.commit_stream(vals, coef, width, tree);
     r.se(ntt_stage);
     r.sb(merkle_stage);
   } else {
     {
-      BigSection big(r.c, st, BIG_NTT);
+      const bool handoff = r.c->sched_handoff && !pl.log_r && !pl.log_s;
+      BigSection big(r, BIG_NTT);
       r.sb(ntt_stage);
-      r.tf.commit_ntt(vals, coef, lde, width);
+      r.tf.commit_ntt(vals, coef, lde, width, handoff ? r.sl.ntt_tail : nullptr);
       r.se(ntt_stage);
+      if (handoff) big.release_behind(r.sl.ntt_tail, r.sl.ntt_done);
     }
     hash_sections(r, lde, width, tree, merkle_stage);
   }
@@ -444,7 +468,7 @@
 }
 
 static void stage_aux(const Run& r, const u64 betas[2], const u64 gammas[2]) {
-  BigSection big(r.c, r.st, BIG_EXCL);
+  BigSection big(r, BIG_EXCL);
   r.sb(ST_AUX);
   aux_build(r.pl.sh, r.ws.tvals, r.pl.N, betas, gammas, r.ws.avals, r.ws.scr, r.ws.err, r.st);
   r.se(ST_AUX);
@@ -455,7 +479,7 @@
   const Workspace& ws = r.ws;
   hipStream_t st = r.st;
   const size_t N = pl.N, M2 = pl.M2, BK = pl.BK, WROWS = pl.WROWS;
-  BigSection big(r.c, st, BIG_NTT);
+  BigSection big(r, BIG_NTT);
   r.sb(ST_QUOTIENT);
   QPointTables wpt;
   wpt.x = ws.wpt;
@@ -495,7 +519,7 @@
   if (pl.stream) {
     quotient_over_windows(r, betas, gammas);
   } else {
-    BigSection big(r.c, st, BIG_EXCL);
+    BigSection big(r, BIG_EXCL);
     r.sb(ST_QUOTIENT);
     QArgs QA;
     quotient_fill_args(QA, pl.sh, ws.tlde, ws.alde, ws.W, ws.mzt, r.pt, betas, gammas, pl.log_n, ws.qv, ws.qpart);
@@ -525,7 +549,7 @@
   const int W = pl.W, A = pl.A, NQ = ProofPlan::NQ, NSPL = pl.NSPL;
   const size_t R = pl.R, NH = pl.NH;
   {
-    BigSection big(r.c, st, BIG_EXCL);
+    BigSection big(r, BIG_EXCL);
     r.sb(ST_OPENINGS);
     u64* d_otab = ws.open + pl.n_part();
     fri_opening_tables(pl.log_r, pl.log_s ? gl2_mul(zeta, zeta) : zeta, pl.log_s ? gl2_mul(zeta_next, zeta_next) : zeta_next, d_otab, st);
@@ -622,7 +646,7 @@
   hipStream_t st = r.st;
   CHK(hipMemcpyAsync(ws.apow, f.apow.data(), f.apow.size() * 4, hipMemcpyHostToDevice, st));
   CHK(hipStreamSynchronize(st));
-  BigSection big(r.c, st, BIG_EXCL);
+  BigSection big(r, BIG_EXCL);
   r.sb(ST_FRI);
   fri_combine_coeffs(pl.sh, ws.tcoef, ws.acoef, ws.qcoef, ws.apow, pl.N, ws.comb, st);
   r.tf.lde(ws.comb, ws.comb + (size_t)6 * pl.N, 6);
@@ -858,6 +882,8 @@
     sl.events.resize(2 * ST_COUNT);
     for (auto& e : sl.events) CHK(hipEventCreate(&e));
   }
+  if (!sl.ntt_tail) CHK(hipEventCreateWithFlags(&sl.ntt_tail, hipEventDisableTiming));
+  if (!sl.ntt_done) CHK(hipEventCreateWithFlags(&sl.ntt_done, hipEventDisableTiming));
   const Run r{c, sl, st, pl, ws, tf, pt};
   const int CAPW = ProofPlan::CAPW;
   ProofParts pp;
diff --git a/plonky2_bn254_amd/lib.py b/plonky2_bn254_amd/lib.py
--- a/plonky2_bn254_amd/lib.py
+++ b/plonky2_bn254_amd/lib.py
@@ -126,6 +126,11 @@
     if hasattr(lib, "bn254s_selftest_proof_plan"):
         lib.bn254s_selftest_proof_plan.argtypes = [C.c_int, C.c_size_t, C.POINTER(Params), C.c_uint64, C.c_int, C.c_int, C.c_int,
                                                    C.c_int, vp, C.c_char_p, C.c_size_t]
+    if hasattr(lib, "bn254s_selftest_big_sched"):
+        lib.bn254s_sched_log.argtypes = [vp, vp, C.c_size_t]
+        lib.bn254s_sched_log.restype = C.c_size_t
+        lib.bn254s_sched_stats.argtypes = [vp, vp]
+        lib.bn254s_selftest_big_sched.argtypes = [vp, vp, C.c_size_t, vp, C.c_size_t, C.POINTER(C.c_size_t), vp]
     lib.bn254s_bench_copy.argtypes = [vp, C.c_size_t, C.c_int]
     lib.bn254s_bench_leafhash.argtypes = [vp, C.c_size_t, C.c_int, C.c_int, C.POINTER(C.c_float)]
     lib.bn254s_g1_generate_trace.argtypes = [vp, vp, vp, vp, C.c_size_t, C.c_uint32, vp, vp]
@@ -255,6 +260,19 @@
     def _check(self, rc, what):
         if rc != 0:
             raise RuntimeError(f"{what} failed with {rc}: {self._lib.bn254s_last_error(self._h).decode()}")
+
+    def sched_log(self):
+        out = np.zeros((512, 8), np.float64)
+        k = self._lib.bn254s_sched_log(self._h, out.ctypes.data_as(C.c_void_p), 512)
+        return [dict(cls=int(r[0]), slot=int(r[1]), begin=float(r[2]), end=float(r[3]), id=int(r[4]),
+                     behind=None if r[5] < 0 else int(r[5]), used=int(r[6])) for r in out[:k]]
+
+    def sched_stats(self) -> dict:
+        out = np.zeros(8, np.uint64)
+        self._check(self._lib.bn254s_sched_stats(self._h, _ptr(out)), "bn254s_sched_stats")
+        v = [int(w) for w in out]
+        return dict(sections=dict(zip(SCHED_CLASSES, v[:4])), early_releases=v[4], behind_event=v[5], max_used=v[6],
+                    handoff=bool(v[7]))
 
     def prove_g1(self, scalars, x, offset, params: Optional[Params] = None) -> Proof:
         params = params or default_params()
@@ -838,6 +856,24 @@
     return None if t is None else t.decode()
 
 
+SCHED_CLASSES = ("ntt", "excl", "hash", "hash_part")
+
+
+def big_sched_script(script, cap=12, cost=(12, 2, 4, 2), fifo=True, convoy=4):
+    lib = load_library()
+    policy = np.array([cap, *cost, int(fifo), convoy], np.int32)
+    sc = np.ascontiguousarray(np.array(script, np.int32).reshape(-1, 2))
+    n = sc.shape[0]
+    adm = np.zeros((max(n, 1), 2), np.uint64)
+    after = np.zeros(max(n, 1), np.uint32)
+    k = C.c_size_t()
+    rc = lib.bn254s_selftest_big_sched(policy.ctypes.data_as(C.c_void_p), sc.ctypes.data_as(C.c_void_p), n, _ptr(adm), adm.shape[0],
+                                       C.byref(k), after.ctypes.data_as(C.c_void_p))
+    if rc != 0:
+        raise ValueError(f"bn254s_selftest_big_sched failed with {rc}")
+    return [(int(a), int(b) - 1 if b else None) for a, b in adm[:k.value]], [int(v) for v in after[:n]]
+
+
 PLAN_BUFFERS = ("in", "tvals", "tcoef", "hist", "tmp", "ldechunk", "sponge", "comb", "tlde", "trees", "avals", "acoef", "alde",
                 "scratch", "quot", "tabs", "open", "fri", "fritrees", "qout", "win")
 _PLAN_HEAD = ("kind", "n", "W", "A", "K", "point_words", "N", "log_n", "log_s", "log_r", "R", "NH", "NSPL", "stream", "lowmem",
```

Result: no change. 90.98 proofs/s, median of 2 (-0.0%).
